# daniel05155/Reinforcement-Learning-in-Music-Generation

Measured on AMD Instinct MI355X. Metric: CW-tokens/sec pretrain fwd+bwd @T=1024, higher is better.
Workload: dtype bf16; 1 GPU; agent_pretrain step (fwd+bwd+clip+Adam), repo dims 512/12/8/2048, synthetic CW tokens (B=512/GPU, T=1024, 7 fields -> 6); per_gpu_batch=512, global_batch=512, seq_len=1024, parallelism=dp1, params=38982227, gemm_table=True

## Files before the change

reinforcement-learning-in-music-generation_amd/csrc/cla_bf16.hip:

```cpp
#include "cwlt_common.h"
#include "cwlt_mfma_bf16.h"

namespace cwlt {
namespace b16 {

__device__ __forceinline__ float phi(float x) { return x > 0.f ? x + 1.f : __expf(x); }
__device__ __forceinline__ float dphi(float x) { return x > 0.f ? 1.f : __expf(x); }
constexpr int FIN_FLOATS = 65 * 64;
__device__ __forceinline__ int stream_of_block(int b, int N, int H) {
    if (N & 7) return b;
    const int x = b & 7, j = b >> 3;
    return ((j / H) * 8 + x) * H + j % H;
}

__device__ __forceinline__ f32x16 load_tile(const float* t, int lane) {
    f32x16 x;
#pragma unroll
    for (int r = 0; r < 16; ++r) x[r] = t[r * 64 + lane];
    return x;
}
__device__ __forceinline__ void store_tile(float* t, int lane, const f32x16& x) {
#pragma unroll
    for (int r = 0; r < 16; ++r) t[r * 64 + lane] = x[r];
}

template <bool STATE_ONLY>
__global__ __launch_bounds__(256) void cla_fwd_bf16_kernel(const bf16_t* __restrict__ q, const bf16_t* __restrict__ k,
                                                           const bf16_t* __restrict__ v, bf16_t* __restrict__ o,
                                                           float* __restrict__ zinv, int H, int L, long ldq, long ldk,
                                                           long ldv, long ldo, float eps, int P, int cps,
                                                           const float* __restrict__ pre, float* __restrict__ part,
                                                           float* __restrict__ fin) {
    __shared__ __attribute__((aligned(16))) bf16_t qs[C * LD];
    __shared__ __attribute__((aligned(16))) bf16_t ks[C * LD];
    __shared__ __attribute__((aligned(16))) bf16_t vs[C * LD];
    __shared__ __attribute__((aligned(16))) bf16_t as_[C * LD];
    __shared__ __attribute__((aligned(16))) float os[C * LDO];
    __shared__ float dens[2][C];

    const int tid = threadIdx.x, lane = tid & 63;
    const int w = __builtin_amdgcn_readfirstlane(tid >> 6);
    const int wi = w >> 1, wj = w & 1;
    const int l31 = lane & 31, hf = lane >> 5;
    const int seg = blockIdx.x % P;
    const int sid = P == 1 ? stream_of_block(blockIdx.x, gridDim.x / H, H) : blockIdx.x / P;
    const int n = sid / H, h = sid % H;
    const bf16_t* qb = q + ((long)n * L) * ldq + h * D;
    const bf16_t* kb = k + ((long)n * L) * ldk + h * D;
    const bf16_t* vb = v + ((long)n * L) * ldv + h * D;
    bf16_t* ob = o + ((long)n * L) * ldo + h * D;
    float* zb = zinv + ((long)n * L) * H + h;

    const int srow = tid >> 3, scol = (tid & 7) * 8;
    const int nch = (L + C - 1) / C;
    const int cbeg = seg * cps, cend = min(nch, cbeg + cps);
    if (cbeg >= nch || (STATE_ONLY && seg == P - 1)) return;
    uint4 rq[2], rk[2], rv[2];
    const bf16x8 ones0 = ones_if(l31 == 0);

    const __amdgpu_buffer_rsrc_t qr = make_rsrc(qb, (uint32_t)(((long)(L - 1) * ldq + D) * 2));
    const __amdgpu_buffer_rsrc_t kr = make_rsrc(kb, (uint32_t)(((long)(L - 1) * ldk + D) * 2));
    const __amdgpu_buffer_rsrc_t vr = make_rsrc(vb, (uint32_t)(((long)(L - 1) * ldv + D) * 2));
#define CLA_LOAD(c)                                                                      \
    _Pragma("unroll") for (int it = 0; it < 2; ++it) {                                   \
        const uint32_t row = (uint32_t)(c) * C + srow + 32 * it;                         \
        if (!STATE_ONLY) rq[it] = buf_load16(qr, (row * (uint32_t)ldq + scol) * 2);      \
        rk[it] = buf_load16(kr, (row * (uint32_t)ldk + scol) * 2);                       \
        rv[it] = buf_load16(vr, (row * (uint32_t)ldv + scol) * 2);                       \
    }
#define CLA_STORE(c)                                                                     \
    _Pragma("unroll") for (int it = 0; it < 2; ++it) {                                   \
        const int row = srow + 32 * it;                                                  \
        const long grow = (long)(c) * C + row;                                           \
        if (grow < L) {                                                                  \
            const float z = 1.0f / (dens[0][row] + dens[1][row] + eps);                  \
            const float4 a = *reinterpret_cast<const float4*>(os + row * LDO + scol);    \
            const float4 b = *reinterpret_cast<const float4*>(os + row * LDO + scol + 4);\
            const float x[8] = {a.x * z, a.y * z, a.z * z, a.w * z, b.x * z, b.y * z, b.z * z, b.w * z}; \
            *reinterpret_cast<uint4*>(ob + grow * ldo + scol) = pack8(x);                \
            if ((tid & 7) == 0) zb[grow * H] = z;                                        \
        }                                                                                \
    }

    CLA_LOAD(cbeg);
    f32x16 S0 = zero16(), S1 = zero16();
    f32x16 Sa = zero16();
    if (!STATE_ONLY && pre && seg > 0) {
        const float* t = pre + (((long)sid * P + seg) * 2 + wj) * (3 * 1024);
        S0 = load_tile(t, lane);
        S1 = load_tile(t + 1024, lane);
        Sa = load_tile(t + 2048, lane);
    }

    for (int c = cbeg; c < cend; ++c) {
        if (!STATE_ONLY && c > cbeg) { CLA_STORE(c - 1); }
#pragma unroll
        for (int it = 0; it < 2; ++it) {
            const int row = srow + 32 * it;
            const bool ok = c * C + row < L;
            float x[8];
            if (!STATE_ONLY) {
                unpack8(rq[it], x);
#pragma unroll
                for (int j = 0; j < 8; ++j) x[j] = ok ? phi(x[j]) : 0.f;
                put_row(qs, row, scol, pack8(x));
            }
            unpack8(rk[it], x);
#pragma unroll
            for (int j = 0; j < 8; ++j) x[j] = ok ? phi(x[j]) : 0.f;
            put_row(ks, row, scol, pack8(x));
            put_row(vs, row, scol, rv[it]);
        }
        __syncthreads();
        if (c + 1 < cend) { CLA_LOAD(c + 1); }

        if (!STATE_ONLY) {
        if (!(wi == 0 && wj == 1)) {
            const f32x16 AT = prod_rows(zero16(), ks, 32 * wj + l31, qs, 32 * wi + l31, 0, 4, hf);
            put_acc_T(as_, 32 * wi + l31, 32 * wj, AT, hf, 0, wi == wj ? l31 : 64, 0.f);
        }
        __syncthreads();

        {
            f32x16 O = zero16(), Oa = zero16();
            const int nks = wi == 0 ? 2 : 4;
#pragma unroll 2
            for (int s = 0; s < nks; ++s) {
                const bf16x8 b = row8(as_, 32 * wi + l31, 16 * s + 8 * hf);
                O = mfma(tfrag8(vs, 16 * s, 32 * wj, lane), b, O);
                if (wj == 0) Oa = mfma(ones0, b, Oa);
            }
#pragma unroll
            for (int t = 0; t < 2; ++t) {
                const f32x16& S = t == 0 ? S0 : S1;
#pragma unroll
                for (int s = 0; s < 2; ++s) {
                    bf16x8 hi, lo;
                    acc_frag(S, s, hi, lo);
                    const bf16x8 b = perm8(qs, 32 * wi + l31, 32 * t + 16 * s, hf);
                    O = mfma_hl(hi, lo, b, O);
                    if (t == wj) {
                        acc_frag(Sa, s, hi, lo);
                        Oa = mfma_hl(hi, lo, b, Oa);
                    }
                }
            }
            put_acc_T_f32(os, 32 * wi + l31, 32 * wj, O, hf);
            if (hf == 0) dens[wj][32 * wi + l31] = Oa[0];
        }
        }
#pragma unroll 2
        for (int s = STATE_ONLY ? 2 * wi : 0; s < (STATE_ONLY ? 2 * wi + 2 : 4); ++s) {
            const bf16x8 b = tfrag8(vs, 16 * s, 32 * wj, lane);
            const bf16x8 a0 = tfrag8(ks, 16 * s, 0, lane);
            const bf16x8 a1 = tfrag8(ks, 16 * s, 32, lane);
            S0 = mfma(a0, b, S0);
            S1 = mfma(a1, b, S1);
            Sa = mfma(wj == 0 ? a0 : a1, ones_if(l31 == 0), Sa);
        }
        __syncthreads();
    }
    if (STATE_ONLY) {
        float* t = part + (((long)sid * P + seg) * 4 + w) * (3 * 1024);
        store_tile(t, lane, S0);
        store_tile(t + 1024, lane, S1);
        store_tile(t + 2048, lane, Sa);
        return;
    }
    CLA_STORE(cend - 1);
#undef CLA_LOAD
#undef CLA_STORE
    if (fin) {
        __syncthreads();
        if (wi == 0) {
            put_acc_T_f32(os, 32 * wj + l31, 0, S0, hf);
            put_acc_T_f32(os, 32 * wj + l31, 32, S1, hf);
            if (l31 == 0) {
#pragma unroll
                for (int r = 0; r < 16; ++r) dens[0][32 * wj + acc_row(r, hf)] = Sa[r];
            }
        }
        __syncthreads();
        float* f = fin + (long)sid * FIN_FLOATS;
#pragma unroll
        for (int it = 0; it < 4; ++it) {
            const int row = (tid >> 4) + 16 * it, col = (tid & 15) * 4;
            *reinterpret_cast<float4*>(f + row * 64 + col) = *reinterpret_cast<const float4*>(os + row * LDO + col);
        }
        if (tid < 64) f[64 * 64 + tid] = dens[0][tid];
    }
}

__global__ __launch_bounds__(256) void seg_prefix_kernel(const float* __restrict__ part, float* __restrict__ pre,
                                                         long total, int P, int NT, int nfwd) {
    const long i = (long)blockIdx.x * 256 + threadIdx.x;
    if (i >= total) return;
    const int e = (int)(i & 1023);
    const int tile = (int)((i >> 10) % NT);
    const int wj = (int)((i >> 10) / NT) & 1;
    const long sid = (i >> 10) / NT / 2;
    const long pstride = (long)4 * NT * 1024, ostride = (long)2 * NT * 1024;
    const float* a = part + sid * P * pstride + ((long)wj * NT + tile) * 1024 + e;
    const float* b = a + (long)2 * NT * 1024;
    float* o = pre + sid * P * ostride + ((long)wj * NT + tile) * 1024 + e;
    float run = 0.f;
    if (tile < nfwd) {
        for (int p = 0; p < P; ++p) {
            o[p * ostride] = run;
            if (p < P - 1) run += a[p * pstride] + b[p * pstride];
        }
    } else {
        for (int p = P - 1; p >= 0; --p) {
            o[p * ostride] = run;
            if (p > 0) run += a[p * pstride] + b[p * pstride];
        }
    }
}

__device__ __forceinline__ uint4 stage_g(uint4 rdo, uint4 ro, float z, float& dden) {
    float a[8], b[8];
    unpack8(rdo, a);
    unpack8(ro, b);
    float dot = 0.f;
#pragma unroll
    for (int j = 0; j < 8; ++j) {
        dot = fmaf(a[j], b[j], dot);
        a[j] *= z;
    }
    dot += dpp_move<0xB1>(dot);
    dot += dpp_move<0x4E>(dot);
    dot += dpp_move<0x141>(dot);
    dden = -dot * z;
    return pack8(a);
}

__device__ __forceinline__ void colsum_store(float (&bsum)[8], float* scratch, float* dst, int tid, int lane, int w) {
    __syncthreads();
#pragma unroll
    for (int j = 0; j < 8; ++j) {
        float v = bsum[j];
        v += __shfl_xor(v, 8, 64);
        v += __shfl_xor(v, 16, 64);
        v += __shfl_xor(v, 32, 64);
        if ((lane >> 3) == 0) scratch[w * 64 + (lane & 7) * 8 + j] = v;
    }
    __syncthreads();
    if (tid < 64) dst[tid] = (scratch[tid] + scratch[64 + tid]) + (scratch[128 + tid] + scratch[192 + tid]);
}

template <bool HAS_DDEN>
__global__ __launch_bounds__(256) void cla_bwd_dq_bf16_kernel(
    const bf16_t* __restrict__ q, const bf16_t* __restrict__ k, const bf16_t* __restrict__ v,
    const bf16_t* __restrict__ out, const bf16_t* __restrict__ dout, const float* __restrict__ zinv,
    const float* __restrict__ dden_in, bf16_t* __restrict__ dq, float* __restrict__ csum, int H, int L, long ldq,
    long ldk, long ldv, long ldo, long lddo, long lddq, int P, int cps, const float* __restrict__ pre) {
    __shared__ __attribute__((aligned(16))) bf16_t gs[C * LD];
    __shared__ __attribute__((aligned(16))) bf16_t vs[C * LD];
    __shared__ __attribute__((aligned(16))) bf16_t ks[C * LD];
    __shared__ __attribute__((aligned(16))) bf16_t ws[C * LD];
    __shared__ __attribute__((aligned(16))) float os[C * LDO];
    __shared__ float dd[C];

    const int tid = threadIdx.x, lane = tid & 63;
    const int w = __builtin_amdgcn_readfirstlane(tid >> 6);
    const int wi = w >> 1, wj = w & 1;
    const int l31 = lane & 31, hf = lane >> 5;
    const int sid = blockIdx.x / P, seg = blockIdx.x % P;
    const int n = sid / H, h = sid % H;
    const bf16_t* qb = q + ((long)n * L) * ldq + h * D;
    const bf16_t* kb = k + ((long)n * L) * ldk + h * D;
    const bf16_t* vb = v + ((long)n * L) * ldv + h * D;
    const bf16_t* ob = out + ((long)n * L) * ldo + h * D;
    const bf16_t* gb = dout + ((long)n * L) * lddo + h * D;
    const float* zb = zinv + ((long)n * L) * H + h;
    const float* ddb = HAS_DDEN ? dden_in + ((long)n * L) * H + h : zb;
    bf16_t* dqb = dq + ((long)n * L) * lddq + h * D;

    const int srow = tid >> 3, scol = (tid & 7) * 8;
    const int nch = (L + C - 1) / C;
    const int cbeg = seg * cps, cend = min(nch, cbeg + cps);
    if (cbeg >= nch) return;
    uint4 rq[2], rk[2], rv[2], rg[2], ro[2], rqp[2];
    float rz[2], rdd[2];

    const __amdgpu_buffer_rsrc_t qr = make_rsrc(qb, (uint32_t)(((long)(L - 1) * ldq + D) * 2));
    const __amdgpu_buffer_rsrc_t kr = make_rsrc(kb, (uint32_t)(((long)(L - 1) * ldk + D) * 2));
    const __amdgpu_buffer_rsrc_t vr = make_rsrc(vb, (uint32_t)(((long)(L - 1) * ldv + D) * 2));
    const __amdgpu_buffer_rsrc_t gr = make_rsrc(gb, (uint32_t)(((long)(L - 1) * lddo + D) * 2));
    const __amdgpu_buffer_rsrc_t orr = make_rsrc(ob, (uint32_t)(((long)(L - 1) * ldo + D) * 2));
    const __amdgpu_buffer_rsrc_t zr = make_rsrc(zb, (uint32_t)(((long)(L - 1) * H + 1) * 4));
    const __amdgpu_buffer_rsrc_t ddr = make_rsrc(ddb, (uint32_t)(((long)(L - 1) * H + 1) * 4));
#define CLA_LOAD(c)                                                                      \
    _Pragma("unroll") for (int it = 0; it < 2; ++it) {                                   \
        const uint32_t row = (uint32_t)(c) * C + srow + 32 * it;                         \
        rq[it] = buf_load16(qr, (row * (uint32_t)ldq + scol) * 2);                       \
        rk[it] = buf_load16(kr, (row * (uint32_t)ldk + scol) * 2);                       \
        rv[it] = buf_load16(vr, (row * (uint32_t)ldv + scol) * 2);                       \
        rg[it] = buf_load16(gr, (row * (uint32_t)lddo + scol) * 2);                      \
        rz[it] = __builtin_bit_cast(float, __builtin_amdgcn_raw_buffer_load_b32(zr, (int)(row * (uint32_t)H * 4), 0, 0)); \
        if (HAS_DDEN)                                                                    \
            rdd[it] = __builtin_bit_cast(float, __builtin_amdgcn_raw_buffer_load_b32(ddr, (int)(row * (uint32_t)H * 4), 0, 0)); \
        else                                                                             \
            ro[it] = buf_load16(orr, (row * (uint32_t)ldo + scol) * 2);                  \
    }
#define CLA_STORE(c)                                                                     \
    _Pragma("unroll") for (int it = 0; it < 2; ++it) {                                   \
        const int row = srow + 32 * it;                                                  \
        const long grow = (long)(c) * C + row;                                           \
        if (grow < L) {                                                                  \
            const float4 a = *reinterpret_cast<const float4*>(os + row * LDO + scol);    \
            const float4 b = *reinterpret_cast<const float4*>(os + row * LDO + scol + 4);\
            float x[8];                                                                  \
            unpack8(rqp[it], x);                                                         \
            x[0] = a.x * dphi(x[0]); x[1] = a.y * dphi(x[1]); x[2] = a.z * dphi(x[2]);   \
            x[3] = a.w * dphi(x[3]); x[4] = b.x * dphi(x[4]); x[5] = b.y * dphi(x[5]);   \
            x[6] = b.z * dphi(x[6]); x[7] = b.w * dphi(x[7]);                            \
            _Pragma("unroll") for (int j = 0; j < 8; ++j) bsum[j] += x[j];               \
            *reinterpret_cast<uint4*>(dqb + grow * lddq + scol) = pack8(x);              \
        }                                                                                \
    }

    float bsum[8];
#pragma unroll
    for (int j = 0; j < 8; ++j) bsum[j] = 0.f;
    CLA_LOAD(cbeg);
    f32x16 T0 = zero16(), T1 = zero16();
    f32x16 Ta = zero16();
    if (pre && seg > 0) {
        const float* t = pre + (((long)sid * P + seg) * 2 + wj) * (8 * 1024);
        T0 = load_tile(t, lane);
        T1 = load_tile(t + 1024, lane);
        Ta = load_tile(t + 2048, lane);
    }
    const bf16x8 ones0 = ones_if(l31 == 0);

    for (int c = cbeg; c < cend; ++c) {
        if (c > cbeg) { CLA_STORE(c - 1); }
#pragma unroll
        for (int it = 0; it < 2; ++it) {
            const int row = srow + 32 * it;
            const bool ok = c * C + row < L;
            float dden;
            uint4 gp;
            if (HAS_DDEN) {
                float a[8];
                unpack8(rg[it], a);
#pragma unroll
                for (int j = 0; j < 8; ++j) a[j] *= rz[it];
                gp = pack8(a);
                dden = rdd[it];
            } else {
                gp = stage_g(rg[it], ro[it], rz[it], dden);
            }
            if ((tid & 7) == 0) dd[row] = dden;
            put_row(gs, row, scol, gp);
            put_row(vs, row, scol, rv[it]);
            float x[8];
            unpack8(rk[it], x);
#pragma unroll
            for (int j = 0; j < 8; ++j) x[j] = ok ? phi(x[j]) : 0.f;
            put_row(ks, row, scol, pack8(x));
            rqp[it] = rq[it];
        }
        __syncthreads();
        if (c + 1 < cend) { CLA_LOAD(c + 1); }

        const float dden_i = dd[32 * wi + l31];
        if (!(wi == 0 && wj == 1)) {
            const f32x16 WT = prod_rows(zero16(), vs, 32 * wj + l31, gs, 32 * wi + l31, 0, 4, hf);
            put_acc_T(ws, 32 * wi + l31, 32 * wj, WT, hf, 0, wi == wj ? l31 : 64, dden_i);
        }
        __syncthreads();

        {
            f32x16 Q = zero16();
            const int nks = wi == 0 ? 2 : 4;
#pragma unroll 2
            for (int s = 0; s < nks; ++s)
                Q = mfma(tfrag8(ks, 16 * s, 32 * wj, lane), row8(ws, 32 * wi + l31, 16 * s + 8 * hf), Q);
            Q = prod_accA(Q, T0, T1, gs, 32 * wi + l31, hf);
            {
                bf16x8 hi, lo;
                acc_frag(Ta, 0, hi, lo);
                const bf16x8 b = first_if(hf == 0, dden_i);
                Q = mfma_hl(hi, lo, b, Q);
            }
            put_acc_T_f32(os, 32 * wi + l31, 32 * wj, Q, hf);
        }
#pragma unroll 2
        for (int s = 0; s < 4; ++s) {
            const bf16x8 b = tfrag8(ks, 16 * s, 32 * wj, lane);
            T0 = mfma(tfrag8(vs, 16 * s, 0, lane), b, T0);
            T1 = mfma(tfrag8(vs, 16 * s, 32, lane), b, T1);
            Ta = mfma(ones0, b, Ta);
        }
        __syncthreads();
    }
    CLA_STORE(cend - 1);
#undef CLA_LOAD
#undef CLA_STORE
    if (csum) colsum_store(bsum, os, csum + (((long)n * P + seg) * H + h) * D, tid, lane, w);
}

template <bool STATE_ONLY>
__global__ __launch_bounds__(256, 2) void cla_bwd_dkdv_bf16_kernel(
    const bf16_t* __restrict__ q, const bf16_t* __restrict__ k, const bf16_t* __restrict__ v,
    const bf16_t* __restrict__ out, const bf16_t* __restrict__ dout, const float* __restrict__ zinv,
    bf16_t* __restrict__ dk, bf16_t* __restrict__ dv, float* __restrict__ csum_k, float* __restrict__ csum_v,
    float* __restrict__ dden_out, int H, int L, long ldq, long ldk, long ldv, long ldo, long lddo, long lddk,
    long lddv, int P, int cps, const float* __restrict__ pre, float* __restrict__ part) {
    __shared__ __attribute__((aligned(16))) bf16_t qs[C * LD];
    __shared__ __attribute__((aligned(16))) bf16_t ks[C * LD];
    __shared__ __attribute__((aligned(16))) bf16_t vs[C * LD];
    __shared__ __attribute__((aligned(16))) bf16_t gs[C * LD];
    __shared__ __attribute__((aligned(16))) bf16_t wt[C * LD];
    __shared__ __attribute__((aligned(16))) bf16_t at[C * LD];
    __shared__ __attribute__((aligned(16))) bf16_t ok_[C * LD];
    __shared__ __attribute__((aligned(16))) bf16_t ov[C * LD];
    __shared__ float dd[C];

    const int tid = threadIdx.x, lane = tid & 63;
    const int w = __builtin_amdgcn_readfirstlane(tid >> 6);
    const int wi = w >> 1, wj = w & 1;
    const int l31 = lane & 31, hf = lane >> 5;
    const int sid = blockIdx.x / P, seg = blockIdx.x % P;
    const int n = sid / H, h = sid % H;
    const bf16_t* qb = q + ((long)n * L) * ldq + h * D;
    const bf16_t* kb = k + ((long)n * L) * ldk + h * D;
    const bf16_t* vb = v + ((long)n * L) * ldv + h * D;
    const bf16_t* ob = out + ((long)n * L) * ldo + h * D;
    const bf16_t* gb = dout + ((long)n * L) * lddo + h * D;
    const float* zb = zinv + ((long)n * L) * H + h;
    bf16_t* dkb = dk + ((long)n * L) * lddk + h * D;
    bf16_t* dvb = dv + ((long)n * L) * lddv + h * D;
    float* ddb = dden_out ? dden_out + ((long)n * L) * H + h : nullptr;

    const int srow = tid >> 3, scol = (tid & 7) * 8;
    const int nch = (L + C - 1) / C;
    const int cbeg = seg * cps, cend = min(nch, cbeg + cps);
    if (cbeg >= nch) return;
    uint4 rq[2], rk[2], rv[2], rg[2], ro[2];
    float rz[2];

    const __amdgpu_buffer_rsrc_t qr = make_rsrc(qb, (uint32_t)(((long)(L - 1) * ldq + D) * 2));
    const __amdgpu_buffer_rsrc_t kr = make_rsrc(kb, (uint32_t)(((long)(L - 1) * ldk + D) * 2));
    const __amdgpu_buffer_rsrc_t vr = make_rsrc(vb, (uint32_t)(((long)(L - 1) * ldv + D) * 2));
    const __amdgpu_buffer_rsrc_t gr = make_rsrc(gb, (uint32_t)(((long)(L - 1) * lddo + D) * 2));
    const __amdgpu_buffer_rsrc_t orr = make_rsrc(ob, (uint32_t)(((long)(L - 1) * ldo + D) * 2));
    const __amdgpu_buffer_rsrc_t zr = make_rsrc(zb, (uint32_t)(((long)(L - 1) * H + 1) * 4));
#define CLA_LOAD(c)                                                                      \
    _Pragma("unroll") for (int it = 0; it < 2; ++it) {                                   \
        const uint32_t row = (uint32_t)(c) * C + srow + 32 * it;                         \
        rq[it] = buf_load16(qr, (row * (uint32_t)ldq + scol) * 2);                       \
        rk[it] = buf_load16(kr, (row * (uint32_t)ldk + scol) * 2);                       \
        rv[it] = buf_load16(vr, (row * (uint32_t)ldv + scol) * 2);                       \
        rg[it] = buf_load16(gr, (row * (uint32_t)lddo + scol) * 2);                      \
        ro[it] = buf_load16(orr, (row * (uint32_t)ldo + scol) * 2);                      \
        rz[it] = __builtin_bit_cast(float, __builtin_amdgcn_raw_buffer_load_b32(zr, (int)(row * (uint32_t)H * 4), 0, 0)); \
    }
#define CLA_STORE(c)                                                                     \
    _Pragma("unroll") for (int it = 0; it < 2; ++it) {                                   \
        const int row = srow + 32 * it;                                                  \
        const long grow = (long)(c) * C + row;                                           \
        if (grow < L) {                                                                  \
            float x[8], f[8];                                                            \
            unpack8(*reinterpret_cast<const uint4*>(ok_ + row * LD + scol), x);          \
            unpack8(*reinterpret_cast<const uint4*>(ks + row * LD + scol), f);           \
            _Pragma("unroll") for (int j = 0; j < 8; ++j) x[j] *= fminf(f[j], 1.0f);     \
            _Pragma("unroll") for (int j = 0; j < 8; ++j) bsk[j] += x[j];                \
            *reinterpret_cast<uint4*>(dkb + grow * lddk + scol) = pack8(x);              \
            const uint4 vv = *reinterpret_cast<const uint4*>(ov + row * LD + scol);      \
            unpack8(vv, f);                                                              \
            _Pragma("unroll") for (int j = 0; j < 8; ++j) bsv[j] += f[j];                \
            *reinterpret_cast<uint4*>(dvb + grow * lddv + scol) = vv;                    \
        }                                                                                \
    }

    float bsk[8], bsv[8];
#pragma unroll
    for (int j = 0; j < 8; ++j) bsk[j] = bsv[j] = 0.f;

    CLA_LOAD(cend - 1);
    f32x16 RT0 = zero16(), RT1 = zero16();
    f32x16 RTa = zero16();
    f32x16 R20 = zero16(), R21 = zero16();
    f32x16 T0 = zero16(), T1 = zero16(), Ta = zero16();
    const bf16x8 ones0 = ones_if(l31 == 0);
    if (!STATE_ONLY && pre && seg < P - 1) {
        const float* t = pre + (((long)sid * P + seg) * 2 + wj) * (8 * 1024) + 3 * 1024;
        RT0 = load_tile(t, lane);
        RT1 = load_tile(t + 1024, lane);
        RTa = load_tile(t + 2048, lane);
        R20 = load_tile(t + 3072, lane);
        R21 = load_tile(t + 4096, lane);
    }

    for (int c = cend - 1; c >= cbeg; --c) {
        if (!STATE_ONLY && c < cend - 1) { CLA_STORE(c + 1); }
#pragma unroll
        for (int it = 0; it < 2; ++it) {
            const int row = srow + 32 * it;
            const bool ok = c * C + row < L;
            float dden;
            const uint4 gp = stage_g(rg[it], ro[it], rz[it], dden);
            if ((tid & 7) == 0) {
                dd[row] = dden;
                if (!STATE_ONLY && ddb && ok) ddb[((long)c * C + row) * H] = dden;
            }
            put_row(gs, row, scol, gp);
            put_row(vs, row, scol, rv[it]);
            float x[8];
            unpack8(rk[it], x);
#pragma unroll
            for (int j = 0; j < 8; ++j) x[j] = ok ? phi(x[j]) : 0.f;
            put_row(ks, row, scol, pack8(x));
            unpack8(rq[it], x);
#pragma unroll
            for (int j = 0; j < 8; ++j) x[j] = ok ? phi(x[j]) : 0.f;
            put_row(qs, row, scol, pack8(x));
        }
        __syncthreads();
        if (c > cbeg) { CLA_LOAD(c - 1); }

        if (!STATE_ONLY) {
        if (!(wi == 0 && wj == 1)) {
            f32x16 W = prod_rows(zero16(), gs, 32 * wi + l31, vs, 32 * wj + l31, 0, 4, hf);
            W = mfma(first_if(hf == 0, dd[32 * wi + l31]), first_if(hf == 0, 1.0f), W);
            put_acc_T(wt, 32 * wj + l31, 32 * wi, W, hf, wi == wj ? l31 : 0, 64, 0.f);
            const f32x16 A = prod_rows(zero16(), qs, 32 * wi + l31, ks, 32 * wj + l31, 0, 4, hf);
            put_acc_T(at, 32 * wj + l31, 32 * wi, A, hf, wi == wj ? l31 : 0, 64, 0.f);
        }
        __syncthreads();

        {
            const int s0 = wi == 1 ? 2 : 0;
            f32x16 K = zero16();
#pragma unroll 2
            for (int s = s0; s < 4; ++s)
                K = mfma(tfrag8(qs, 16 * s, 32 * wj, lane), row8(wt, 32 * wi + l31, 16 * s + 8 * hf), K);
            K = prod_accA(K, RT0, RT1, vs, 32 * wi + l31, hf);
            {
                bf16x8 hi, lo;
                acc_frag(RTa, 0, hi, lo);
                const bf16x8 b = first_if(hf == 0, 1.0f);
                K = mfma_hl(hi, lo, b, K);
            }
            put_acc_T(ok_, 32 * wi + l31, 32 * wj, K, hf, 0, 64, 0.f);
            f32x16 V = zero16();
#pragma unroll 2
            for (int s = s0; s < 4; ++s)
                V = mfma(tfrag8(gs, 16 * s, 32 * wj, lane), row8(at, 32 * wi + l31, 16 * s + 8 * hf), V);
            V = prod_accA(V, R20, R21, ks, 32 * wi + l31, hf);
            put_acc_T(ov, 32 * wi + l31, 32 * wj, V, hf, 0, 64, 0.f);
        }
        }
#pragma unroll 2
        for (int s = STATE_ONLY ? 2 * wi : 0; s < (STATE_ONLY ? 2 * wi + 2 : 4); ++s) {
            const bf16x8 g0 = tfrag8(gs, 16 * s, 0, lane), g1 = tfrag8(gs, 16 * s, 32, lane);
            const bf16x8 q0 = tfrag8(qs, 16 * s, 0, lane), q1 = tfrag8(qs, 16 * s, 32, lane);
            const bf16x8 bq = wj == 0 ? q0 : q1;
            const bf16x8 bg = wj == 0 ? g0 : g1;
            RT0 = mfma(g0, bq, RT0);
            RT1 = mfma(g1, bq, RT1);
            R20 = mfma(q0, bg, R20);
            R21 = mfma(q1, bg, R21);
            bf16x8 dh, dl;
#pragma unroll
            for (int j = 0; j < 8; ++j) {
                const float x = l31 == 0 ? dd[16 * s + 8 * hf + j] : 0.f;
                const __bf16 hh = (__bf16)x;
                dh[j] = hh;
                dl[j] = (__bf16)(x - (float)hh);
            }
            RTa = mfma(dh, bq, RTa);
            RTa = mfma(dl, bq, RTa);
            if (STATE_ONLY) {
                const bf16x8 bk = tfrag8(ks, 16 * s, 32 * wj, lane);
                T0 = mfma(tfrag8(vs, 16 * s, 0, lane), bk, T0);
                T1 = mfma(tfrag8(vs, 16 * s, 32, lane), bk, T1);
                Ta = mfma(ones0, bk, Ta);
            }
        }
        __syncthreads();
    }
    if (STATE_ONLY) {
        float* t = part + (((long)sid * P + seg) * 4 + w) * (8 * 1024);
        store_tile(t, lane, T0);
        store_tile(t + 1024, lane, T1);
        store_tile(t + 2048, lane, Ta);
        store_tile(t + 3072, lane, RT0);
        store_tile(t + 4096, lane, RT1);
        store_tile(t + 5120, lane, RTa);
        store_tile(t + 6144, lane, R20);
        store_tile(t + 7168, lane, R21);
        return;
    }
    CLA_STORE(cbeg);
#undef CLA_LOAD
#undef CLA_STORE
    if (csum_k) {
        float* scratch = reinterpret_cast<float*>(wt);
        colsum_store(bsk, scratch, csum_k + (((long)n * P + seg) * H + h) * D, tid, lane, w);
        colsum_store(bsv, scratch, csum_v + (((long)n * P + seg) * H + h) * D, tid, lane, w);
    }
}

struct ChunkRegs {
    uint4 q, k, v, g, o;
    float z;
};

__device__ __forceinline__ float min1(float f) { return __builtin_amdgcn_fmed3f(f, 0.0f, 1.0f); }

__device__ __forceinline__ void put_acc_T_dphi(bf16_t* x, const bf16_t* f_t, int xrow, int c0, const f32x16& acc, int hf) {
#pragma unroll
    for (int g = 0; g < 4; ++g) {
        const uint2 fr = *reinterpret_cast<const uint2*>(f_t + xrow * LD + c0 + 8 * g + 4 * hf);
        const float f0 = __uint_as_float(fr.x << 16), f1 = __uint_as_float(fr.x & 0xffff0000u);
        const float f2 = __uint_as_float(fr.y << 16), f3 = __uint_as_float(fr.y & 0xffff0000u);
        bf16x4 p;
        p[0] = (__bf16)(acc[4 * g] * min1(f0));
        p[1] = (__bf16)(acc[4 * g + 1] * min1(f1));
        p[2] = (__bf16)(acc[4 * g + 2] * min1(f2));
        p[3] = (__bf16)(acc[4 * g + 3] * min1(f3));
        *reinterpret_cast<uint2*>(x + xrow * LD + c0 + 8 * g + 4 * hf) = __builtin_bit_cast(uint2, p);
    }
}
__device__ __forceinline__ void put_acc_T_all(bf16_t* x, int xrow, int c0, const f32x16& acc, int hf) {
#pragma unroll
    for (int g = 0; g < 4; ++g) {
        bf16x4 p;
#pragma unroll
        for (int u = 0; u < 4; ++u) p[u] = (__bf16)acc[4 * g + u];
        *reinterpret_cast<uint2*>(x + xrow * LD + c0 + 8 * g + 4 * hf) = __builtin_bit_cast(uint2, p);
    }
}
__device__ __forceinline__ void put_acc_T_ge(bf16_t* x, int xrow, int c0, const f32x16& acc, int hf, int lo) {
#pragma unroll
    for (int g = 0; g < 4; ++g) {
        bf16x4 p;
#pragma unroll
        for (int u = 0; u < 4; ++u) p[u] = (__bf16)(8 * g + 4 * hf + u >= lo ? acc[4 * g + u] : 0.f);
        *reinterpret_cast<uint2*>(x + xrow * LD + c0 + 8 * g + 4 * hf) = __builtin_bit_cast(uint2, p);
    }
}
__device__ __forceinline__ f32x16 prod_rows4(const bf16_t* a_t, int arow, const bf16_t* b_t, int brow, int hf) {
    f32x16 acc = mfma(row8(a_t, arow, 8 * hf), row8(b_t, brow, 8 * hf), zero16());
#pragma unroll
    for (int s = 1; s < 4; ++s) acc = mfma(row8(a_t, arow, 16 * s + 8 * hf), row8(b_t, brow, 16 * s + 8 * hf), acc);
    return acc;
}
__device__ __forceinline__ bf16x8 negate8(bf16x8 x) {
    uint4 u = __builtin_bit_cast(uint4, x);
    u.x ^= 0x80008000u; u.y ^= 0x80008000u; u.z ^= 0x80008000u; u.w ^= 0x80008000u;
    return __builtin_bit_cast(bf16x8, u);
}

__global__ __launch_bounds__(512, 1) void cla_bwd_sweep_bf16_kernel(
    const bf16_t* __restrict__ q, const bf16_t* __restrict__ k, const bf16_t* __restrict__ v,
    const bf16_t* __restrict__ out, const bf16_t* __restrict__ dout, const float* __restrict__ zinv,
    const float* __restrict__ fin, bf16_t* __restrict__ dq, bf16_t* __restrict__ dk, bf16_t* __restrict__ dv,
    float* __restrict__ csum_q, float* __restrict__ csum_k, float* __restrict__ csum_v, int H, int L, long ldq,
    long ldk, long ldv, long ldo, long lddo, long lddq, long lddk, long lddv) {
    constexpr int TILE = C * LD;
    __shared__ __attribute__((aligned(16))) bf16_t in_[2 * 4 * TILE];
    __shared__ __attribute__((aligned(16))) bf16_t er[2 * TILE];
    __shared__ __attribute__((aligned(16))) bf16_t es[TILE];
    __shared__ __attribute__((aligned(16))) bf16_t wt[TILE];
    __shared__ __attribute__((aligned(16))) bf16_t at[TILE];
    __shared__ __attribute__((aligned(16))) bf16_t ok_[TILE];
    __shared__ __attribute__((aligned(16))) bf16_t ov[TILE];
    __shared__ __attribute__((aligned(16))) bf16_t oq[TILE];
    __shared__ float dd[2][C];
    __shared__ float r1s[2][C];
    __shared__ float ksm[C];

    const int tid = threadIdx.x, lane = tid & 63;
    const int w8 = __builtin_amdgcn_readfirstlane(tid >> 6);
    const bool kvg = w8 < 4;
    const int w = w8 & 3, wi = w >> 1, wj = w & 1;
    const int l31 = lane & 31, hf = lane >> 5;
    const int sid = stream_of_block(blockIdx.x, gridDim.x / H, H);
    const int n = sid / H, h = sid % H;
    const bf16_t* qb = q + ((long)n * L) * ldq + h * D;
    const bf16_t* kb = k + ((long)n * L) * ldk + h * D;
    const bf16_t* vb = v + ((long)n * L) * ldv + h * D;
    const bf16_t* ob = out + ((long)n * L) * ldo + h * D;
    const bf16_t* gb = dout + ((long)n * L) * lddo + h * D;
    const float* zb = zinv + ((long)n * L) * H + h;
    bf16_t* dqb = dq + ((long)n * L) * lddq + h * D;
    bf16_t* dkb = dk + ((long)n * L) * lddk + h * D;
    bf16_t* dvb = dv + ((long)n * L) * lddv + h * D;

    const int srow = tid >> 3, scol = (tid & 7) * 8;
    const int orow = (tid & 255) >> 3;
    const int nch = (L + C - 1) / C;

    const __amdgpu_buffer_rsrc_t qr = make_rsrc(qb, (uint32_t)(((long)(L - 1) * ldq + D) * 2));
    const __amdgpu_buffer_rsrc_t kr = make_rsrc(kb, (uint32_t)(((long)(L - 1) * ldk + D) * 2));
    const __amdgpu_buffer_rsrc_t vr = make_rsrc(vb, (uint32_t)(((long)(L - 1) * ldv + D) * 2));
    const __amdgpu_buffer_rsrc_t gr = make_rsrc(gb, (uint32_t)(((long)(L - 1) * lddo + D) * 2));
    const __amdgpu_buffer_rsrc_t orr = make_rsrc(ob, (uint32_t)(((long)(L - 1) * ldo + D) * 2));
    const __amdgpu_buffer_rsrc_t zr = make_rsrc(zb, (uint32_t)(((long)(L - 1) * H + 1) * 4));

    auto load = [&](ChunkRegs& R, int c) __attribute__((always_inline)) {
        const uint32_t row = (uint32_t)c * C + srow;
        R.q = buf_load16(qr, (row * (uint32_t)ldq + scol) * 2);
        R.k = buf_load16(kr, (row * (uint32_t)ldk + scol) * 2);
        R.v = buf_load16(vr, (row * (uint32_t)ldv + scol) * 2);
        R.g = buf_load16(gr, (row * (uint32_t)lddo + scol) * 2);
        R.o = buf_load16(orr, (row * (uint32_t)ldo + scol) * 2);
        R.z = __builtin_bit_cast(float, __builtin_amdgcn_raw_buffer_load_b32(zr, (int)(row * (uint32_t)H * 4), 0, 0));
    };
    auto stage = [&](const ChunkRegs& R, int c, int b) __attribute__((always_inline)) {
        bf16_t* t = in_ + b * 4 * TILE;
        float dden;
        const uint4 gp = stage_g(R.g, R.o, R.z, dden);
        put_row(t + 3 * TILE, srow, scol, gp);
        if ((tid & 7) == 0) {
            dd[b][srow] = dden;
            const __bf16 hh = (__bf16)dden;
            const __bf16 ll = (__bf16)(dden - (float)hh);
            const uint32_t hl = (uint32_t)__builtin_bit_cast(unsigned short, hh) |
                                ((uint32_t)__builtin_bit_cast(unsigned short, ll) << 16);
            put_row(t + 3 * TILE, srow, 64, make_uint4(hl, 0u, 0u, 0u));
        }
        put_row(t + 2 * TILE, srow, scol, R.v);
        float x[8], y[8];
        unpack8(R.k, x);
        unpack8(R.q, y);
#pragma unroll
        for (int j = 0; j < 8; ++j) {
            x[j] = phi(x[j]);
            y[j] = phi(y[j]);
        }
        if ((c + 1) * C > L && c * C + srow >= L) {
#pragma unroll
            for (int j = 0; j < 8; ++j) x[j] = y[j] = 0.f;
        }
        put_row(t + 1 * TILE, srow, scol, pack8(x));
        put_row(t, srow, scol, pack8(y));
    };

    typedef float f32x8 __attribute__((ext_vector_type(8)));
    f32x8 bs0 = 0.f, bs1 = 0.f;
    auto widen = [](uint4 r) __attribute__((always_inline)) {
        f32x8 x;
        x[0] = __uint_as_float(r.x << 16); x[1] = __uint_as_float(r.x & 0xffff0000u);
        x[2] = __uint_as_float(r.y << 16); x[3] = __uint_as_float(r.y & 0xffff0000u);
        x[4] = __uint_as_float(r.z << 16); x[5] = __uint_as_float(r.z & 0xffff0000u);
        x[6] = __uint_as_float(r.w << 16); x[7] = __uint_as_float(r.w & 0xffff0000u);
        return x;
    };
    const bf16_t* t0 = kvg ? ok_ : oq;
    bf16_t* g0 = kvg ? dkb : dqb;
    const long l0 = kvg ? lddk : lddq;
    auto store = [&](int c, f32x8& b0, f32x8& b1) __attribute__((always_inline)) {
#pragma unroll
        for (int it = 0; it < 2; ++it) {
            const int row = orow + 32 * it;
            const long grow = (long)c * C + row;
            if (grow < L) {
                const uint4 a = *reinterpret_cast<const uint4*>(t0 + row * LD + scol);
                b0 += widen(a);
                *reinterpret_cast<uint4*>(g0 + grow * l0 + scol) = a;
                if (kvg) {
                    const uint4 b = *reinterpret_cast<const uint4*>(ov + row * LD + scol);
                    b1 += widen(b);
                    *reinterpret_cast<uint4*>(dvb + grow * lddv + scol) = b;
                }
            }
        }
    };

    f32x16 st = zero16(), sa = zero16();
    if (!kvg) {
        const float* f = fin + (long)sid * FIN_FLOATS;
#pragma unroll
        for (int r = 0; r < 16; ++r) st[r] = f[(32 * wi + acc_row(r, hf)) * 64 + 32 * wj + l31];
        if (wi == 0) sa[0] = hf == 0 ? f[64 * 64 + 32 * wj + l31] : 0.f;
    } else {
        put_acc_T_all(er, 32 * wj + l31, 32 * wi, st, hf);
        if (wi == 0 && hf == 0) r1s[0][32 * wj + l31] = 0.f;
    }
    const bf16x8 ones0 = ones_if(l31 == 0);
    const bf16x8 one0 = first_if(hf == 0, 1.0f);

    auto iter = [&](int c, ChunkRegs& R, const int b) __attribute__((always_inline)) {
        if (c < nch - 1) store(c + 1, bs0, bs1);
        if (c >= 1) {
            stage(R, c - 1, 1 - b);
            if (c >= 3) load(R, c - 3);
        }
        const bf16_t* qs = in_ + b * 4 * TILE;
        const bf16_t* ks = qs + TILE;
        const bf16_t* vs = qs + 2 * TILE;
        const bf16_t* gs = qs + 3 * TILE;
        const float dden_i = dd[b][32 * wi + l31];
        __builtin_amdgcn_sched_barrier(0);
        if (kvg) {
            if (!(wi == 0 && wj == 1)) {
                f32x16 W = prod_rows4(gs, 32 * wi + l31, vs, 32 * wj + l31, hf);
                W = mfma(first_if(hf == 0, dden_i), one0, W);
                if (wi == wj) put_acc_T_ge(wt, 32 * wj + l31, 32 * wi, W, hf, l31);
                else put_acc_T_all(wt, 32 * wj + l31, 32 * wi, W, hf);
            }
            __builtin_amdgcn_sched_barrier(0);
#pragma unroll
            for (int s = 0; s < 4; ++s) {
                const bf16x8 bq = tfrag8(qs, 16 * s, 32 * wj, lane);
                st = mfma(tfrag8(gs, 16 * s, 32 * wi, lane), bq, st);
                if (wi == 0) sa = mfma(tfrag8(gs, 16 * s, 64, lane), bq, sa);
            }
            if (c > 0) {
                put_acc_T_all(er + (1 - b) * TILE, 32 * wj + l31, 32 * wi, st, hf);
                if (wi == 0 && hf == 0) r1s[1 - b][32 * wj + l31] = sa[0] + sa[1];
            }
        } else {
            if (!(wi == 0 && wj == 1)) {
                const f32x16 A = prod_rows4(qs, 32 * wi + l31, ks, 32 * wj + l31, hf);
                if (wi == wj) put_acc_T_ge(at, 32 * wj + l31, 32 * wi, A, hf, l31);
                else put_acc_T_all(at, 32 * wj + l31, 32 * wi, A, hf);
            }
            __builtin_amdgcn_sched_barrier(0);
            if (c == 0) {
                st = zero16();
                sa = zero16();
            } else {
#pragma unroll
                for (int s = 0; s < 4; ++s) {
                    const bf16x8 nb = negate8(tfrag8(ks, 16 * s, 32 * wj, lane));
                    st = mfma(tfrag8(vs, 16 * s, 32 * wi, lane), nb, st);
                    if (wi == 0) sa = mfma(ones0, nb, sa);
                }
            }
            put_acc_T_all(es, 32 * wj + l31, 32 * wi, st, hf);
            if (wi == 0 && hf == 0) ksm[32 * wj + l31] = sa[0];
        }
        __syncthreads();
        if (kvg) {
            const bf16_t* rs = er + b * TILE;
            f32x16 K = prod_rows4(rs, 32 * wj + l31, vs, 32 * wi + l31, hf);
            K = mfma(first_if(hf == 0, r1s[b][32 * wj + l31]), one0, K);
            f32x16 V = mfma(tfrag8(rs, 0, 32 * wj, lane), row8(ks, 32 * wi + l31, 8 * hf), zero16());
#pragma unroll
            for (int s = 1; s < 4; ++s)
                V = mfma(tfrag8(rs, 16 * s, 32 * wj, lane), row8(ks, 32 * wi + l31, 16 * s + 8 * hf), V);
            __builtin_amdgcn_sched_barrier(0);
            if (wi == 0) {
#pragma unroll
                for (int s = 0; s < 2; ++s) {
                    K = mfma(tfrag8(qs, 16 * s, 32 * wj, lane), row8(wt, 32 * wi + l31, 16 * s + 8 * hf), K);
                    V = mfma(tfrag8(gs, 16 * s, 32 * wj, lane), row8(at, 32 * wi + l31, 16 * s + 8 * hf), V);
                }
            }
#pragma unroll
            for (int s = 2; s < 4; ++s) {
                K = mfma(tfrag8(qs, 16 * s, 32 * wj, lane), row8(wt, 32 * wi + l31, 16 * s + 8 * hf), K);
                V = mfma(tfrag8(gs, 16 * s, 32 * wj, lane), row8(at, 32 * wi + l31, 16 * s + 8 * hf), V);
            }
            __builtin_amdgcn_sched_barrier(0);
            put_acc_T_dphi(ok_, ks, 32 * wi + l31, 32 * wj, K, hf);
            put_acc_T_all(ov, 32 * wi + l31, 32 * wj, V, hf);
        } else {
            f32x16 Q = prod_rows4(es, 32 * wj + l31, gs, 32 * wi + l31, hf);
            Q = mfma(first_if(hf == 0, ksm[32 * wj + l31]), first_if(hf == 0, dden_i), Q);
            __builtin_amdgcn_sched_barrier(0);
#pragma unroll
            for (int s = 0; s < 2; ++s)
                Q = mfma(tfrag8(ks, 16 * s, 32 * wj, lane), tfrag8(wt, 16 * s, 32 * wi, lane), Q);
            if (wi == 1) {
#pragma unroll
                for (int s = 2; s < 4; ++s)
                    Q = mfma(tfrag8(ks, 16 * s, 32 * wj, lane), tfrag8(wt, 16 * s, 32 * wi, lane), Q);
            }
            put_acc_T_dphi(oq, qs, 32 * wi + l31, 32 * wj, Q, hf);
        }
        __syncthreads();
    };

    ChunkRegs RA, RB;
    load(RA, nch - 1);
    if (nch > 1) load(RB, nch - 2);
    stage(RA, nch - 1, 0);
    if (nch > 2) load(RA, nch - 3);
    __syncthreads();
    for (int c = nch - 1; c >= 0; c -= 2) {
        iter(c, RB, 0);
        if (c >= 1) iter(c - 1, RA, 1);
    }
    store(0, bs0, bs1);

    if (csum_q) {
        float* scratch = reinterpret_cast<float*>(wt);
        __syncthreads();
#pragma unroll
        for (int j = 0; j < 8; ++j) {
            float x = bs0[j], y = bs1[j];
            x += __shfl_xor(x, 8, 64);
            y += __shfl_xor(y, 8, 64);
            x += __shfl_xor(x, 16, 64);
            y += __shfl_xor(y, 16, 64);
            x += __shfl_xor(x, 32, 64);
            y += __shfl_xor(y, 32, 64);
            if ((lane >> 3) == 0) {
                scratch[((kvg ? 1 : 0) * 4 + w) * 64 + (lane & 7) * 8 + j] = x;
                if (kvg) scratch[(2 * 4 + w) * 64 + (lane & 7) * 8 + j] = y;
            }
        }
        __syncthreads();
        if (tid < 192) {
            const int a = tid >> 6, e = tid & 63;
            const float s = (scratch[(a * 4 + 0) * 64 + e] + scratch[(a * 4 + 1) * 64 + e]) +
                            (scratch[(a * 4 + 2) * 64 + e] + scratch[(a * 4 + 3) * 64 + e]);
            float* dst = a == 0 ? csum_q : a == 1 ? csum_k : csum_v;
            dst[(long)sid * D + e] = s;
        }
    }
}

}

int scan_segments(int N, int H, int L) {
    const long streams = (long)N * H;
    const int nch = (L + b16::C - 1) / b16::C;
    if (streams >= 256 || nch < 4) return 1;
    long want = (512 + streams - 1) / streams;
    if (want > 16) want = 16;
    if (want > nch / 2) want = nch / 2;
    if (want < 2) return 1;
    const int cps = (nch + (int)want - 1) / (int)want;
    return (nch + cps - 1) / cps;
}
static int seg_cps(int L, int P) { return (((L + b16::C - 1) / b16::C) + P - 1) / P; }

long scan_seg_floats(int N, int H, int P, int backward) {
    return P > 1 ? (long)N * H * P * 6 * (backward ? 8 : 3) * 1024 : 0;
}

long scan_final_state_floats(int N, int H) { return (long)N * H * b16::FIN_FLOATS; }

int launch_cla_fwd_bf16(const void* q, const void* k, const void* v, void* out, float* zinv, int N, int H, int L,
                        long ldq, long ldk, long ldv, long ldo, float eps, int P, float* ws, float* fin,
                        hipStream_t st) {
    const int nch = (L + b16::C - 1) / b16::C;
    if (P <= 1) {
        hipLaunchKernelGGL(b16::cla_fwd_bf16_kernel<false>, dim3(N * H), dim3(256), 0, st, (const bf16_t*)q,
                           (const bf16_t*)k, (const bf16_t*)v, (bf16_t*)out, zinv, H, L, ldq, ldk, ldv, ldo, eps, 1, nch,
                           (const float*)nullptr, (float*)nullptr, fin);
        return (int)hipGetLastError();
    }
    const int cps = seg_cps(L, P);
    const long NS = (long)N * H;
    float* part = ws;
    float* pre = ws + NS * P * 4 * 3 * 1024;
    hipLaunchKernelGGL(b16::cla_fwd_bf16_kernel<true>, dim3(NS * P), dim3(256), 0, st, (const bf16_t*)q,
                       (const bf16_t*)k, (const bf16_t*)v, (bf16_t*)out, zinv, H, L, ldq, ldk, ldv, ldo, eps, P, cps,
                       (const float*)nullptr, part, (float*)nullptr);
    const long total = NS * 2 * 3 * 1024;
    hipLaunchKernelGGL(b16::seg_prefix_kernel, dim3((unsigned)((total + 255) / 256)), dim3(256), 0, st, part, pre, total,
                       P, 3, 3);
    hipLaunchKernelGGL(b16::cla_fwd_bf16_kernel<false>, dim3(NS * P), dim3(256), 0, st, (const bf16_t*)q,
                       (const bf16_t*)k, (const bf16_t*)v, (bf16_t*)out, zinv, H, L, ldq, ldk, ldv, ldo, eps, P, cps,
                       (const float*)pre, (float*)nullptr, (float*)nullptr);
    return (int)hipGetLastError();
}

int launch_cla_bwd_sweep_bf16(const void* q, const void* k, const void* v, const void* out, const float* zinv,
                              const void* dout, const float* fin, void* dq, void* dk, void* dv, float* csum_q,
                              float* csum_k, float* csum_v, int N, int H, int L, long ldq, long ldk, long ldv, long ldo,
                              long lddo, long lddq, long lddk, long lddv, hipStream_t st) {
    hipLaunchKernelGGL(b16::cla_bwd_sweep_bf16_kernel, dim3(N * H), dim3(512), 0, st, (const bf16_t*)q,
                       (const bf16_t*)k, (const bf16_t*)v, (const bf16_t*)out, (const bf16_t*)dout, zinv, fin,
                       (bf16_t*)dq, (bf16_t*)dk, (bf16_t*)dv, csum_q, csum_k, csum_v, H, L, ldq, ldk, ldv, ldo, lddo,
                       lddq, lddk, lddv);
    return (int)hipGetLastError();
}

int launch_cla_bwd_dq_bf16(const void* q, const void* k, const void* v, const void* out, const float* zinv,
                           const void* dout, const float* dden, void* dq, float* csum, int N, int H, int L, long ldq,
                           long ldk, long ldv, long ldo, long lddo, long lddq, int P, float* ws, hipStream_t st) {
    const int nch = (L + b16::C - 1) / b16::C;
    const long NS = (long)N * H;
    const int cps = P > 1 ? seg_cps(L, P) : nch;
    const float* pre = P > 1 ? ws + NS * P * 4 * 8 * 1024 : nullptr;
    if (P < 1) P = 1;
    if (dden)
        hipLaunchKernelGGL(b16::cla_bwd_dq_bf16_kernel<true>, dim3(NS * P), dim3(256), 0, st, (const bf16_t*)q,
                           (const bf16_t*)k, (const bf16_t*)v, (const bf16_t*)out, (const bf16_t*)dout, zinv, dden,
                           (bf16_t*)dq, csum, H, L, ldq, ldk, ldv, ldo, lddo, lddq, P, cps, pre);
    else
        hipLaunchKernelGGL(b16::cla_bwd_dq_bf16_kernel<false>, dim3(NS * P), dim3(256), 0, st, (const bf16_t*)q,
                           (const bf16_t*)k, (const bf16_t*)v, (const bf16_t*)out, (const bf16_t*)dout, zinv, dden,
                           (bf16_t*)dq, csum, H, L, ldq, ldk, ldv, ldo, lddo, lddq, P, cps, pre);
    return (int)hipGetLastError();
}

int launch_cla_bwd_dkdv_bf16(const void* q, const void* k, const void* v, const void* out, const float* zinv,
                             const void* dout, void* dk, void* dv, float* csum_k, float* csum_v, float* dden_out,
                             int N, int H, int L, long ldq, long ldk, long ldv, long ldo, long lddo, long lddk,
                             long lddv, int P, float* ws, hipStream_t st) {
    const int nch = (L + b16::C - 1) / b16::C;
    const long NS = (long)N * H;
    if (P <= 1) {
        hipLaunchKernelGGL(b16::cla_bwd_dkdv_bf16_kernel<false>, dim3(NS), dim3(256), 0, st, (const bf16_t*)q,
                           (const bf16_t*)k, (const bf16_t*)v, (const bf16_t*)out, (const bf16_t*)dout, zinv,
                           (bf16_t*)dk, (bf16_t*)dv, csum_k, csum_v, dden_out, H, L, ldq, ldk, ldv, ldo, lddo, lddk,
                           lddv, 1, nch, (const float*)nullptr, (float*)nullptr);
        return (int)hipGetLastError();
    }
    const int cps = seg_cps(L, P);
    float* part = ws;
    float* pre = ws + NS * P * 4 * 8 * 1024;
    hipLaunchKernelGGL(b16::cla_bwd_dkdv_bf16_kernel<true>, dim3(NS * P), dim3(256), 0, st, (const bf16_t*)q,
                       (const bf16_t*)k, (const bf16_t*)v, (const bf16_t*)out, (const bf16_t*)dout, zinv, (bf16_t*)dk,
                       (bf16_t*)dv, (float*)nullptr, (float*)nullptr, (float*)nullptr, H, L, ldq, ldk, ldv, ldo, lddo,
                       lddk, lddv, P, cps, (const float*)nullptr, part);
    const long total = NS * 2 * 8 * 1024;
    hipLaunchKernelGGL(b16::seg_prefix_kernel, dim3((unsigned)((total + 255) / 256)), dim3(256), 0, st, part, pre, total,
                       P, 8, 3);
    hipLaunchKernelGGL(b16::cla_bwd_dkdv_bf16_kernel<false>, dim3(NS * P), dim3(256), 0, st, (const bf16_t*)q,
                       (const bf16_t*)k, (const bf16_t*)v, (const bf16_t*)out, (const bf16_t*)dout, zinv, (bf16_t*)dk,
                       (bf16_t*)dv, csum_k, csum_v, dden_out, H, L, ldq, ldk, ldv, ldo, lddo, lddk, lddv, P, cps,
                       (const float*)pre, (float*)nullptr);
    return (int)hipGetLastError();
}

}
```

reinforcement-learning-in-music-generation_amd/csrc/cwlt_mfma_bf16.h:

```cpp
#pragma once
#include "cwlt_common.h"

namespace cwlt {
namespace b16 {

constexpr int D = 64;
constexpr int C = 64;
constexpr int LD = 72;
constexpr int LDO = 68;

typedef __bf16 bf16x8 __attribute__((ext_vector_type(8)));
typedef __bf16 bf16x4 __attribute__((ext_vector_type(4)));
typedef short s16x4 __attribute__((ext_vector_type(4)));
typedef __attribute__((address_space(3))) s16x4 lds_s16x4;

__device__ __forceinline__ constexpr int acc_row(int r, int hf) { return (r & 3) + 8 * (r >> 2) + 4 * hf; }

__device__ __forceinline__ f32x16 mfma(bf16x8 a, bf16x8 b, f32x16 c) {
    return __builtin_amdgcn_mfma_f32_32x32x16_bf16(a, b, c, 0, 0, 0);
}
__device__ __forceinline__ f32x16 zero16() {
    f32x16 z;
#pragma unroll
    for (int i = 0; i < 16; ++i) z[i] = 0.f;
    return z;
}

__device__ __forceinline__ bf16x8 row8(const bf16_t* t, int row, int k) {
    return __builtin_bit_cast(bf16x8, *reinterpret_cast<const uint4*>(t + row * LD + k));
}
__device__ __forceinline__ bf16x8 perm8(const bf16_t* t, int row, int k0, int hf) {
    const uint2 a = *reinterpret_cast<const uint2*>(t + row * LD + k0 + 4 * hf);
    const uint2 b = *reinterpret_cast<const uint2*>(t + row * LD + k0 + 8 + 4 * hf);
    return __builtin_bit_cast(bf16x8, make_uint4(a.x, a.y, b.x, b.y));
}
__device__ __forceinline__ bf16x8 tfrag8(const bf16_t* t, int k0, int c0, int lane) {
    const int q = (lane >> 2) & 3, p = lane & 3;
    const bf16_t* base = t + (k0 + 8 * (lane >> 5) + q) * LD + c0 + 16 * ((lane >> 4) & 1) + 4 * p;
    const s16x4 a = __builtin_amdgcn_ds_read_tr16_b64_v4i16((lds_s16x4*)(base));
    const s16x4 b = __builtin_amdgcn_ds_read_tr16_b64_v4i16((lds_s16x4*)(base + 4 * LD));
    return __builtin_bit_cast(bf16x8, __builtin_shufflevector(a, b, 0, 1, 2, 3, 4, 5, 6, 7));
}
#ifndef CWLT_STATE_LO
#define CWLT_STATE_LO 0
#endif
constexpr bool STATE_LO = CWLT_STATE_LO != 0;
__device__ __forceinline__ f32x16 mfma_hl(const bf16x8& hi, const bf16x8& lo, bf16x8 b, f32x16 acc) {
    acc = __builtin_amdgcn_mfma_f32_32x32x16_bf16(hi, b, acc, 0, 0, 0);
    if (STATE_LO) acc = __builtin_amdgcn_mfma_f32_32x32x16_bf16(lo, b, acc, 0, 0, 0);
    return acc;
}
__device__ __forceinline__ void acc_frag(const f32x16& S, int s, bf16x8& hi, bf16x8& lo) {
#pragma unroll
    for (int j = 0; j < 8; ++j) {
        const float x = S[8 * s + j];
        const __bf16 h = (__bf16)x;
        hi[j] = h;
        lo[j] = (__bf16)(x - (float)h);
    }
}
__device__ __forceinline__ bf16x8 first_if(bool c, float x) {
    bf16x8 v;
#pragma unroll
    for (int j = 0; j < 8; ++j) v[j] = (__bf16)0.0f;
    v[0] = (__bf16)(c ? x : 0.0f);
    return v;
}
__device__ __forceinline__ bf16x8 ones_if(bool c) {
    bf16x8 v;
#pragma unroll
    for (int j = 0; j < 8; ++j) v[j] = (__bf16)(c ? 1.0f : 0.0f);
    return v;
}

__device__ __forceinline__ f32x16 prod_rows(f32x16 acc, const bf16_t* a_t, int arow, const bf16_t* b_t, int brow,
                                            int s0, int s1, int hf) {
#pragma unroll 2
    for (int s = s0; s < s1; ++s)
        acc = mfma(row8(a_t, arow, 16 * s + 8 * hf), row8(b_t, brow, 16 * s + 8 * hf), acc);
    return acc;
}
__device__ __forceinline__ f32x16 prod_accA(f32x16 acc, const f32x16& X0, const f32x16& X1, const bf16_t* b_t,
                                            int brow, int hf) {
#pragma unroll
    for (int t = 0; t < 2; ++t) {
        const f32x16& X = t == 0 ? X0 : X1;
#pragma unroll
        for (int s = 0; s < 2; ++s) {
            bf16x8 hi, lo;
            acc_frag(X, s, hi, lo);
            const bf16x8 b = perm8(b_t, brow, 32 * t + 16 * s, hf);
            acc = mfma_hl(hi, lo, b, acc);
        }
    }
    return acc;
}

__device__ __forceinline__ void unpack8(uint4 r, float (&x)[8]) {
    x[0] = __uint_as_float(r.x << 16); x[1] = __uint_as_float(r.x & 0xffff0000u);
    x[2] = __uint_as_float(r.y << 16); x[3] = __uint_as_float(r.y & 0xffff0000u);
    x[4] = __uint_as_float(r.z << 16); x[5] = __uint_as_float(r.z & 0xffff0000u);
    x[6] = __uint_as_float(r.w << 16); x[7] = __uint_as_float(r.w & 0xffff0000u);
}
__device__ __forceinline__ uint4 pack8(const float (&x)[8]) {
    bf16x8 v;
#pragma unroll
    for (int j = 0; j < 8; ++j) v[j] = (__bf16)x[j];
    return __builtin_bit_cast(uint4, v);
}
__device__ __forceinline__ void put_row(bf16_t* t, int row, int col, uint4 v) {
    *reinterpret_cast<uint4*>(t + row * LD + col) = v;
}
__device__ __forceinline__ void put_acc_T(bf16_t* x, int xrow, int c0, const f32x16& acc, int hf, int lo, int hi,
                                          float add) {
#pragma unroll
    for (int g = 0; g < 4; ++g) {
        bf16x4 p;
#pragma unroll
        for (int u = 0; u < 4; ++u) {
            const int rr = 8 * g + 4 * hf + u;
            p[u] = (__bf16)((rr >= lo && rr <= hi) ? acc[4 * g + u] + add : 0.f);
        }
        *reinterpret_cast<uint2*>(x + xrow * LD + c0 + 8 * g + 4 * hf) = __builtin_bit_cast(uint2, p);
    }
}
__device__ __forceinline__ void put_acc_T_f32(float* x, int xrow, int c0, const f32x16& acc, int hf) {
#pragma unroll
    for (int g = 0; g < 4; ++g)
        *reinterpret_cast<float4*>(x + xrow * LDO + c0 + 8 * g + 4 * hf) =
            make_float4(acc[4 * g], acc[4 * g + 1], acc[4 * g + 2], acc[4 * g + 3]);
}

}
}
```

Baseline: 3.254 million CW-tokens/s.

## Swizzle LDS tiles with XOR layout and software-pipeline MFMA fragment fetches

```diff
diff --git a/reinforcement-learning-in-music-generation_amd/csrc/cla_bf16.hip b/reinforcement-learning-in-music-generation_amd/csrc/cla_bf16.hip
--- a/reinforcement-learning-in-music-generation_amd/csrc/cla_bf16.hip
+++ b/reinforcement-learning-in-music-generation_amd/csrc/cla_bf16.hip
@@ -1,3 +1,5 @@
+#include <type_traits>
+
 #include "cwlt_common.h"
 #include "cwlt_mfma_bf16.h"
 
@@ -31,10 +33,10 @@
                                                            long ldv, long ldo, float eps, int P, int cps,
                                                            const float* __restrict__ pre, float* __restrict__ part,
                                                            float* __restrict__ fin) {
-    __shared__ __attribute__((aligned(16))) bf16_t qs[C * LD];
-    __shared__ __attribute__((aligned(16))) bf16_t ks[C * LD];
-    __shared__ __attribute__((aligned(16))) bf16_t vs[C * LD];
-    __shared__ __attribute__((aligned(16))) bf16_t as_[C * LD];
+    __shared__ __attribute__((aligned(16))) bf16_t qs[sw::TILE];
+    __shared__ __attribute__((aligned(16))) bf16_t ks[sw::TILE];
+    __shared__ __attribute__((aligned(16))) bf16_t vs[sw::TILE];
+    __shared__ __attribute__((aligned(16))) bf16_t as_[sw::TILE];
     __shared__ __attribute__((aligned(16))) float os[C * LDO];
     __shared__ float dens[2][C];
 
@@ -52,6 +54,13 @@
     float* zb = zinv + ((long)n * L) * H + h;
 
     const int srow = tid >> 3, scol = (tid & 7) * 8;
+    int sb = sw::base(srow, scol);
+    int bi8 = sw::base(32 * wi + l31, 8 * hf), bj8 = sw::base(32 * wj + l31, 8 * hf);
+    int bi4 = sw::base(32 * wi + l31, 4 * hf), bj4 = sw::base(32 * wj + l31, 4 * hf);
+    sw::TBase tb = sw::tbase(lane);
+#define CLA_FRESH()                                                                                  \
+    CWLT_SW_FRESH(sb); CWLT_SW_FRESH(bi8); CWLT_SW_FRESH(bj8); CWLT_SW_FRESH(bi4); CWLT_SW_FRESH(bj4); \
+    CWLT_SW_FRESH(tb.b0); CWLT_SW_FRESH(tb.b4)
     const int nch = (L + C - 1) / C;
     const int cbeg = seg * cps, cend = min(nch, cbeg + cps);
     if (cbeg >= nch || (STATE_ONLY && seg == P - 1)) return;
@@ -93,6 +102,7 @@
     }
 
     for (int c = cbeg; c < cend; ++c) {
+        CLA_FRESH();
         if (!STATE_ONLY && c > cbeg) { CLA_STORE(c - 1); }
 #pragma unroll
         for (int it = 0; it < 2; ++it) {
@@ -103,21 +113,21 @@
                 unpack8(rq[it], x);
 #pragma unroll
                 for (int j = 0; j < 8; ++j) x[j] = ok ? phi(x[j]) : 0.f;
-                put_row(qs, row, scol, pack8(x));
+                sw::put_row(qs + 32 * it * sw::ROW, sb, pack8(x));
             }
             unpack8(rk[it], x);
 #pragma unroll
             for (int j = 0; j < 8; ++j) x[j] = ok ? phi(x[j]) : 0.f;
-            put_row(ks, row, scol, pack8(x));
-            put_row(vs, row, scol, rv[it]);
+            sw::put_row(ks + 32 * it * sw::ROW, sb, pack8(x));
+            sw::put_row(vs + 32 * it * sw::ROW, sb, rv[it]);
         }
         __syncthreads();
         if (c + 1 < cend) { CLA_LOAD(c + 1); }
 
         if (!STATE_ONLY) {
         if (!(wi == 0 && wj == 1)) {
-            const f32x16 AT = prod_rows(zero16(), ks, 32 * wj + l31, qs, 32 * wi + l31, 0, 4, hf);
-            put_acc_T(as_, 32 * wi + l31, 32 * wj, AT, hf, 0, wi == wj ? l31 : 64, 0.f);
+            const f32x16 AT = sw::prod_rows(zero16(), ks, bj8, qs, bi8, 0, 4);
+            sw::put_acc_T(as_, bi4, 32 * wj, AT, hf, 0, wi == wj ? l31 : 64, 0.f);
         }
         __syncthreads();
 
@@ -126,8 +136,8 @@
             const int nks = wi == 0 ? 2 : 4;
 #pragma unroll 2
             for (int s = 0; s < nks; ++s) {
-                const bf16x8 b = row8(as_, 32 * wi + l31, 16 * s + 8 * hf);
-                O = mfma(tfrag8(vs, 16 * s, 32 * wj, lane), b, O);
+                const bf16x8 b = sw::row8(as_, bi8, 16 * s);
+                O = mfma(sw::tfrag8(vs, tb, 16 * s, 32 * wj), b, O);
                 if (wj == 0) Oa = mfma(ones0, b, Oa);
             }
 #pragma unroll
@@ -137,7 +147,7 @@
                 for (int s = 0; s < 2; ++s) {
                     bf16x8 hi, lo;
                     acc_frag(S, s, hi, lo);
-                    const bf16x8 b = perm8(qs, 32 * wi + l31, 32 * t + 16 * s, hf);
+                    const bf16x8 b = sw::perm8(qs, bi4, 32 * t + 16 * s);
                     O = mfma_hl(hi, lo, b, O);
                     if (t == wj) {
                         acc_frag(Sa, s, hi, lo);
@@ -151,9 +161,9 @@
         }
 #pragma unroll 2
         for (int s = STATE_ONLY ? 2 * wi : 0; s < (STATE_ONLY ? 2 * wi + 2 : 4); ++s) {
-            const bf16x8 b = tfrag8(vs, 16 * s, 32 * wj, lane);
-            const bf16x8 a0 = tfrag8(ks, 16 * s, 0, lane);
-            const bf16x8 a1 = tfrag8(ks, 16 * s, 32, lane);
+            const bf16x8 b = sw::tfrag8(vs, tb, 16 * s, 32 * wj);
+            const bf16x8 a0 = sw::tfrag8(ks, tb, 16 * s, 0);
+            const bf16x8 a1 = sw::tfrag8(ks, tb, 16 * s, 32);
             S0 = mfma(a0, b, S0);
             S1 = mfma(a1, b, S1);
             Sa = mfma(wj == 0 ? a0 : a1, ones_if(l31 == 0), Sa);
@@ -170,6 +180,7 @@
     CLA_STORE(cend - 1);
 #undef CLA_LOAD
 #undef CLA_STORE
+#undef CLA_FRESH
     if (fin) {
         __syncthreads();
         if (wi == 0) {
@@ -254,10 +265,10 @@
     const bf16_t* __restrict__ out, const bf16_t* __restrict__ dout, const float* __restrict__ zinv,
     const float* __restrict__ dden_in, bf16_t* __restrict__ dq, float* __restrict__ csum, int H, int L, long ldq,
     long ldk, long ldv, long ldo, long lddo, long lddq, int P, int cps, const float* __restrict__ pre) {
-    __shared__ __attribute__((aligned(16))) bf16_t gs[C * LD];
-    __shared__ __attribute__((aligned(16))) bf16_t vs[C * LD];
-    __shared__ __attribute__((aligned(16))) bf16_t ks[C * LD];
-    __shared__ __attribute__((aligned(16))) bf16_t ws[C * LD];
+    __shared__ __attribute__((aligned(16))) bf16_t gs[sw::TILE];
+    __shared__ __attribute__((aligned(16))) bf16_t vs[sw::TILE];
+    __shared__ __attribute__((aligned(16))) bf16_t ks[sw::TILE];
+    __shared__ __attribute__((aligned(16))) bf16_t ws[sw::TILE];
     __shared__ __attribute__((aligned(16))) float os[C * LDO];
     __shared__ float dd[C];
 
@@ -277,6 +288,13 @@
     bf16_t* dqb = dq + ((long)n * L) * lddq + h * D;
 
     const int srow = tid >> 3, scol = (tid & 7) * 8;
+    int sb = sw::base(srow, scol);
+    int bi8 = sw::base(32 * wi + l31, 8 * hf), bj8 = sw::base(32 * wj + l31, 8 * hf);
+    int bi4 = sw::base(32 * wi + l31, 4 * hf), bj4 = sw::base(32 * wj + l31, 4 * hf);
+    sw::TBase tb = sw::tbase(lane);
+#define CLA_FRESH()                                                                                  \
+    CWLT_SW_FRESH(sb); CWLT_SW_FRESH(bi8); CWLT_SW_FRESH(bj8); CWLT_SW_FRESH(bi4); CWLT_SW_FRESH(bj4); \
+    CWLT_SW_FRESH(tb.b0); CWLT_SW_FRESH(tb.b4)
     const int nch = (L + C - 1) / C;
     const int cbeg = seg * cps, cend = min(nch, cbeg + cps);
     if (cbeg >= nch) return;
@@ -335,6 +353,7 @@
     const bf16x8 ones0 = ones_if(l31 == 0);
 
     for (int c = cbeg; c < cend; ++c) {
+        CLA_FRESH();
         if (c > cbeg) { CLA_STORE(c - 1); }
 #pragma unroll
         for (int it = 0; it < 2; ++it) {
@@ -353,13 +372,13 @@
                 gp = stage_g(rg[it], ro[it], rz[it], dden);
             }
             if ((tid & 7) == 0) dd[row] = dden;
-            put_row(gs, row, scol, gp);
-            put_row(vs, row, scol, rv[it]);
+            sw::put_row(gs + 32 * it * sw::ROW, sb, gp);
+            sw::put_row(vs + 32 * it * sw::ROW, sb, rv[it]);
             float x[8];
             unpack8(rk[it], x);
 #pragma unroll
             for (int j = 0; j < 8; ++j) x[j] = ok ? phi(x[j]) : 0.f;
-            put_row(ks, row, scol, pack8(x));
+            sw::put_row(ks + 32 * it * sw::ROW, sb, pack8(x));
             rqp[it] = rq[it];
         }
         __syncthreads();
@@ -367,8 +386,8 @@
 
         const float dden_i = dd[32 * wi + l31];
         if (!(wi == 0 && wj == 1)) {
-            const f32x16 WT = prod_rows(zero16(), vs, 32 * wj + l31, gs, 32 * wi + l31, 0, 4, hf);
-            put_acc_T(ws, 32 * wi + l31, 32 * wj, WT, hf, 0, wi == wj ? l31 : 64, dden_i);
+            const f32x16 WT = sw::prod_rows(zero16(), vs, bj8, gs, bi8, 0, 4);
+            sw::put_acc_T(ws, bi4, 32 * wj, WT, hf, 0, wi == wj ? l31 : 64, dden_i);
         }
         __syncthreads();
 
@@ -377,8 +396,8 @@
             const int nks = wi == 0 ? 2 : 4;
 #pragma unroll 2
             for (int s = 0; s < nks; ++s)
-                Q = mfma(tfrag8(ks, 16 * s, 32 * wj, lane), row8(ws, 32 * wi + l31, 16 * s + 8 * hf), Q);
-            Q = prod_accA(Q, T0, T1, gs, 32 * wi + l31, hf);
+                Q = mfma(sw::tfrag8(ks, tb, 16 * s, 32 * wj), sw::row8(ws, bi8, 16 * s), Q);
+            Q = sw::prod_accA(Q, T0, T1, gs, bi4);
             {
                 bf16x8 hi, lo;
                 acc_frag(Ta, 0, hi, lo);
@@ -389,9 +408,9 @@
         }
 #pragma unroll 2
         for (int s = 0; s < 4; ++s) {
-            const bf16x8 b = tfrag8(ks, 16 * s, 32 * wj, lane);
-            T0 = mfma(tfrag8(vs, 16 * s, 0, lane), b, T0);
-            T1 = mfma(tfrag8(vs, 16 * s, 32, lane), b, T1);
+            const bf16x8 b = sw::tfrag8(ks, tb, 16 * s, 32 * wj);
+            T0 = mfma(sw::tfrag8(vs, tb, 16 * s, 0), b, T0);
+            T1 = mfma(sw::tfrag8(vs, tb, 16 * s, 32), b, T1);
             Ta = mfma(ones0, b, Ta);
         }
         __syncthreads();
@@ -399,6 +418,7 @@
     CLA_STORE(cend - 1);
 #undef CLA_LOAD
 #undef CLA_STORE
+#undef CLA_FRESH
     if (csum) colsum_store(bsum, os, csum + (((long)n * P + seg) * H + h) * D, tid, lane, w);
 }
 
@@ -409,14 +429,14 @@
     bf16_t* __restrict__ dk, bf16_t* __restrict__ dv, float* __restrict__ csum_k, float* __restrict__ csum_v,
     float* __restrict__ dden_out, int H, int L, long ldq, long ldk, long ldv, long ldo, long lddo, long lddk,
     long lddv, int P, int cps, const float* __restrict__ pre, float* __restrict__ part) {
-    __shared__ __attribute__((aligned(16))) bf16_t qs[C * LD];
-    __shared__ __attribute__((aligned(16))) bf16_t ks[C * LD];
-    __shared__ __attribute__((aligned(16))) bf16_t vs[C * LD];
-    __shared__ __attribute__((aligned(16))) bf16_t gs[C * LD];
-    __shared__ __attribute__((aligned(16))) bf16_t wt[C * LD];
-    __shared__ __attribute__((aligned(16))) bf16_t at[C * LD];
-    __shared__ __attribute__((aligned(16))) bf16_t ok_[C * LD];
-    __shared__ __attribute__((aligned(16))) bf16_t ov[C * LD];
+    __shared__ __attribute__((aligned(16))) bf16_t qs[sw::TILE];
+    __shared__ __attribute__((aligned(16))) bf16_t ks[sw::TILE];
+    __shared__ __attribute__((aligned(16))) bf16_t vs[sw::TILE];
+    __shared__ __attribute__((aligned(16))) bf16_t gs[sw::TILE];
+    __shared__ __attribute__((aligned(16))) bf16_t wt[sw::TILE];
+    __shared__ __attribute__((aligned(16))) bf16_t at[sw::TILE];
+    __shared__ __attribute__((aligned(16))) bf16_t ok_[sw::TILE];
+    __shared__ __attribute__((aligned(16))) bf16_t ov[sw::TILE];
     __shared__ float dd[C];
 
     const int tid = threadIdx.x, lane = tid & 63;
@@ -436,6 +456,13 @@
     float* ddb = dden_out ? dden_out + ((long)n * L) * H + h : nullptr;
 
     const int srow = tid >> 3, scol = (tid & 7) * 8;
+    int sb = sw::base(srow, scol);
+    int bi8 = sw::base(32 * wi + l31, 8 * hf), bj8 = sw::base(32 * wj + l31, 8 * hf);
+    int bi4 = sw::base(32 * wi + l31, 4 * hf), bj4 = sw::base(32 * wj + l31, 4 * hf);
+    sw::TBase tb = sw::tbase(lane);
+#define CLA_FRESH()                                                                                  \
+    CWLT_SW_FRESH(sb); CWLT_SW_FRESH(bi8); CWLT_SW_FRESH(bj8); CWLT_SW_FRESH(bi4); CWLT_SW_FRESH(bj4); \
+    CWLT_SW_FRESH(tb.b0); CWLT_SW_FRESH(tb.b4)
     const int nch = (L + C - 1) / C;
     const int cbeg = seg * cps, cend = min(nch, cbeg + cps);
     if (cbeg >= nch) return;
@@ -464,12 +491,12 @@
         const long grow = (long)(c) * C + row;                                           \
         if (grow < L) {                                                                  \
             float x[8], f[8];                                                            \
-            unpack8(*reinterpret_cast<const uint4*>(ok_ + row * LD + scol), x);          \
-            unpack8(*reinterpret_cast<const uint4*>(ks + row * LD + scol), f);           \
+            unpack8(sw::get_row(ok_ + 32 * it * sw::ROW, sb), x);                        \
+            unpack8(sw::get_row(ks + 32 * it * sw::ROW, sb), f);                         \
             _Pragma("unroll") for (int j = 0; j < 8; ++j) x[j] *= fminf(f[j], 1.0f);     \
             _Pragma("unroll") for (int j = 0; j < 8; ++j) bsk[j] += x[j];                \
             *reinterpret_cast<uint4*>(dkb + grow * lddk + scol) = pack8(x);              \
-            const uint4 vv = *reinterpret_cast<const uint4*>(ov + row * LD + scol);      \
+            const uint4 vv = sw::get_row(ov + 32 * it * sw::ROW, sb);                    \
             unpack8(vv, f);                                                              \
             _Pragma("unroll") for (int j = 0; j < 8; ++j) bsv[j] += f[j];                \
             *reinterpret_cast<uint4*>(dvb + grow * lddv + scol) = vv;                    \
@@ -496,6 +523,7 @@
     }
 
     for (int c = cend - 1; c >= cbeg; --c) {
+        CLA_FRESH();
         if (!STATE_ONLY && c < cend - 1) { CLA_STORE(c + 1); }
 #pragma unroll
         for (int it = 0; it < 2; ++it) {
@@ -507,28 +535,28 @@
                 dd[row] = dden;
                 if (!STATE_ONLY && ddb && ok) ddb[((long)c * C + row) * H] = dden;
             }
-            put_row(gs, row, scol, gp);
-            put_row(vs, row, scol, rv[it]);
+            sw::put_row(gs + 32 * it * sw::ROW, sb, gp);
+            sw::put_row(vs + 32 * it * sw::ROW, sb, rv[it]);
             float x[8];
             unpack8(rk[it], x);
 #pragma unroll
             for (int j = 0; j < 8; ++j) x[j] = ok ? phi(x[j]) : 0.f;
-            put_row(ks, row, scol, pack8(x));
+            sw::put_row(ks + 32 * it * sw::ROW, sb, pack8(x));
             unpack8(rq[it], x);
 #pragma unroll
             for (int j = 0; j < 8; ++j) x[j] = ok ? phi(x[j]) : 0.f;
-            put_row(qs, row, scol, pack8(x));
+            sw::put_row(qs + 32 * it * sw::ROW, sb, pack8(x));
         }
         __syncthreads();
         if (c > cbeg) { CLA_LOAD(c - 1); }
 
         if (!STATE_ONLY) {
         if (!(wi == 0 && wj == 1)) {
-            f32x16 W = prod_rows(zero16(), gs, 32 * wi + l31, vs, 32 * wj + l31, 0, 4, hf);
+            f32x16 W = sw::prod_rows(zero16(), gs, bi8, vs, bj8, 0, 4);
             W = mfma(first_if(hf == 0, dd[32 * wi + l31]), first_if(hf == 0, 1.0f), W);
-            put_acc_T(wt, 32 * wj + l31, 32 * wi, W, hf, wi == wj ? l31 : 0, 64, 0.f);
-            const f32x16 A = prod_rows(zero16(), qs, 32 * wi + l31, ks, 32 * wj + l31, 0, 4, hf);
-            put_acc_T(at, 32 * wj + l31, 32 * wi, A, hf, wi == wj ? l31 : 0, 64, 0.f);
+            sw::put_acc_T(wt, bj4, 32 * wi, W, hf, wi == wj ? l31 : 0, 64, 0.f);
+            const f32x16 A = sw::prod_rows(zero16(), qs, bi8, ks, bj8, 0, 4);
+            sw::put_acc_T(at, bj4, 32 * wi, A, hf, wi == wj ? l31 : 0, 64, 0.f);
         }
         __syncthreads();
 
@@ -537,27 +565,27 @@
             f32x16 K = zero16();
 #pragma unroll 2
             for (int s = s0; s < 4; ++s)
-                K = mfma(tfrag8(qs, 16 * s, 32 * wj, lane), row8(wt, 32 * wi + l31, 16 * s + 8 * hf), K);
-            K = prod_accA(K, RT0, RT1, vs, 32 * wi + l31, hf);
+                K = mfma(sw::tfrag8(qs, tb, 16 * s, 32 * wj), sw::row8(wt, bi8, 16 * s), K);
+            K = sw::prod_accA(K, RT0, RT1, vs, bi4);
             {
                 bf16x8 hi, lo;
                 acc_frag(RTa, 0, hi, lo);
                 const bf16x8 b = first_if(hf == 0, 1.0f);
                 K = mfma_hl(hi, lo, b, K);
             }
-            put_acc_T(ok_, 32 * wi + l31, 32 * wj, K, hf, 0, 64, 0.f);
+            sw::put_acc_T(ok_, bi4, 32 * wj, K, hf, 0, 64, 0.f);
             f32x16 V = zero16();
 #pragma unroll 2
             for (int s = s0; s < 4; ++s)
-                V = mfma(tfrag8(gs, 16 * s, 32 * wj, lane), row8(at, 32 * wi + l31, 16 * s + 8 * hf), V);
-            V = prod_accA(V, R20, R21, ks, 32 * wi + l31, hf);
-            put_acc_T(ov, 32 * wi + l31, 32 * wj, V, hf, 0, 64, 0.f);
+                V = mfma(sw::tfrag8(gs, tb, 16 * s, 32 * wj), sw::row8(at, bi8, 16 * s), V);
+            V = sw::prod_accA(V, R20, R21, ks, bi4);
+            sw::put_acc_T(ov, bi4, 32 * wj, V, hf, 0, 64, 0.f);
         }
         }
 #pragma unroll 2
         for (int s = STATE_ONLY ? 2 * wi : 0; s < (STATE_ONLY ? 2 * wi + 2 : 4); ++s) {
-            const bf16x8 g0 = tfrag8(gs, 16 * s, 0, lane), g1 = tfrag8(gs, 16 * s, 32, lane);
-            const bf16x8 q0 = tfrag8(qs, 16 * s, 0, lane), q1 = tfrag8(qs, 16 * s, 32, lane);
+            const bf16x8 g0 = sw::tfrag8(gs, tb, 16 * s, 0), g1 = sw::tfrag8(gs, tb, 16 * s, 32);
+            const bf16x8 q0 = sw::tfrag8(qs, tb, 16 * s, 0), q1 = sw::tfrag8(qs, tb, 16 * s, 32);
             const bf16x8 bq = wj == 0 ? q0 : q1;
             const bf16x8 bg = wj == 0 ? g0 : g1;
             RT0 = mfma(g0, bq, RT0);
@@ -575,9 +603,9 @@
             RTa = mfma(dh, bq, RTa);
             RTa = mfma(dl, bq, RTa);
             if (STATE_ONLY) {
-                const bf16x8 bk = tfrag8(ks, 16 * s, 32 * wj, lane);
-                T0 = mfma(tfrag8(vs, 16 * s, 0, lane), bk, T0);
-                T1 = mfma(tfrag8(vs, 16 * s, 32, lane), bk, T1);
+                const bf16x8 bk = sw::tfrag8(ks, tb, 16 * s, 32 * wj);
+                T0 = mfma(sw::tfrag8(vs, tb, 16 * s, 0), bk, T0);
+                T1 = mfma(sw::tfrag8(vs, tb, 16 * s, 32), bk, T1);
                 Ta = mfma(ones0, bk, Ta);
             }
         }
@@ -598,6 +626,7 @@
     CLA_STORE(cbeg);
 #undef CLA_LOAD
 #undef CLA_STORE
+#undef CLA_FRESH
     if (csum_k) {
         float* scratch = reinterpret_cast<float*>(wt);
         colsum_store(bsk, scratch, csum_k + (((long)n * P + seg) * H + h) * D, tid, lane, w);
@@ -612,10 +641,10 @@
 
 __device__ __forceinline__ float min1(float f) { return __builtin_amdgcn_fmed3f(f, 0.0f, 1.0f); }
 
-__device__ __forceinline__ void put_acc_T_dphi(bf16_t* x, const bf16_t* f_t, int xrow, int c0, const f32x16& acc, int hf) {
+__device__ __forceinline__ void put_acc_T_dphi(bf16_t* x, const bf16_t* f_t, int x4, int c0, const f32x16& acc) {
 #pragma unroll
     for (int g = 0; g < 4; ++g) {
-        const uint2 fr = *reinterpret_cast<const uint2*>(f_t + xrow * LD + c0 + 8 * g + 4 * hf);
+        const uint2 fr = *sw::at<uint2>(f_t, x4, c0 + 8 * g);
         const float f0 = __uint_as_float(fr.x << 16), f1 = __uint_as_float(fr.x & 0xffff0000u);
         const float f2 = __uint_as_float(fr.y << 16), f3 = __uint_as_float(fr.y & 0xffff0000u);
         bf16x4 p;
@@ -623,37 +652,44 @@
         p[1] = (__bf16)(acc[4 * g + 1] * min1(f1));
         p[2] = (__bf16)(acc[4 * g + 2] * min1(f2));
         p[3] = (__bf16)(acc[4 * g + 3] * min1(f3));
-        *reinterpret_cast<uint2*>(x + xrow * LD + c0 + 8 * g + 4 * hf) = __builtin_bit_cast(uint2, p);
-    }
-}
-__device__ __forceinline__ void put_acc_T_all(bf16_t* x, int xrow, int c0, const f32x16& acc, int hf) {
+        *sw::at<uint2>(x, x4, c0 + 8 * g) = __builtin_bit_cast(uint2, p);
+    }
+}
+__device__ __forceinline__ void put_acc_T_all(bf16_t* x, int x4, int c0, const f32x16& acc) {
 #pragma unroll
     for (int g = 0; g < 4; ++g) {
         bf16x4 p;
 #pragma unroll
         for (int u = 0; u < 4; ++u) p[u] = (__bf16)acc[4 * g + u];
-        *reinterpret_cast<uint2*>(x + xrow * LD + c0 + 8 * g + 4 * hf) = __builtin_bit_cast(uint2, p);
-    }
-}
-__device__ __forceinline__ void put_acc_T_ge(bf16_t* x, int xrow, int c0, const f32x16& acc, int hf, int lo) {
+        *sw::at<uint2>(x, x4, c0 + 8 * g) = __builtin_bit_cast(uint2, p);
+    }
+}
+__device__ __forceinline__ void put_acc_T_ge(bf16_t* x, int x4, int c0, const f32x16& acc, int hf, int lo) {
 #pragma unroll
     for (int g = 0; g < 4; ++g) {
         bf16x4 p;
 #pragma unroll
         for (int u = 0; u < 4; ++u) p[u] = (__bf16)(8 * g + 4 * hf + u >= lo ? acc[4 * g + u] : 0.f);
-        *reinterpret_cast<uint2*>(x + xrow * LD + c0 + 8 * g + 4 * hf) = __builtin_bit_cast(uint2, p);
-    }
-}
-__device__ __forceinline__ f32x16 prod_rows4(const bf16_t* a_t, int arow, const bf16_t* b_t, int brow, int hf) {
-    f32x16 acc = mfma(row8(a_t, arow, 8 * hf), row8(b_t, brow, 8 * hf), zero16());
-#pragma unroll
-    for (int s = 1; s < 4; ++s) acc = mfma(row8(a_t, arow, 16 * s + 8 * hf), row8(b_t, brow, 16 * s + 8 * hf), acc);
+        *sw::at<uint2>(x, x4, c0 + 8 * g) = __builtin_bit_cast(uint2, p);
+    }
+}
+__device__ __forceinline__ f32x16 prod_rows4(const bf16_t* a_t, int a8, const bf16_t* b_t, int b8) {
+    f32x16 acc = mfma(sw::row8(a_t, a8, 0), sw::row8(b_t, b8, 0), zero16());
+#pragma unroll
+    for (int s = 1; s < 4; ++s) acc = mfma(sw::row8(a_t, a8, 16 * s), sw::row8(b_t, b8, 16 * s), acc);
     return acc;
 }
 __device__ __forceinline__ bf16x8 negate8(bf16x8 x) {
     uint4 u = __builtin_bit_cast(uint4, x);
     u.x ^= 0x80008000u; u.y ^= 0x80008000u; u.z ^= 0x80008000u; u.w ^= 0x80008000u;
     return __builtin_bit_cast(bf16x8, u);
+}
+
+__device__ __forceinline__ bf16x8 dden_frag(const bf16_t* t, int k0, int lane) {
+    const bf16_t* base = t + (k0 + 8 * (lane >> 5) + ((lane >> 2) & 3)) * 8 + 4 * (lane & 1);
+    const s16x4 a = __builtin_amdgcn_ds_read_tr16_b64_v4i16((lds_s16x4*)(base));
+    const s16x4 b = __builtin_amdgcn_ds_read_tr16_b64_v4i16((lds_s16x4*)(base + 4 * 8));
+    return __builtin_bit_cast(bf16x8, __builtin_shufflevector(a, b, 0, 1, 2, 3, 4, 5, 6, 7));
 }
 
 __global__ __launch_bounds__(512, 1) void cla_bwd_sweep_bf16_kernel(
@@ -662,7 +698,7 @@
     const float* __restrict__ fin, bf16_t* __restrict__ dq, bf16_t* __restrict__ dk, bf16_t* __restrict__ dv,
     float* __restrict__ csum_q, float* __restrict__ csum_k, float* __restrict__ csum_v, int H, int L, long ldq,
     long ldk, long ldv, long ldo, long lddo, long lddq, long lddk, long lddv) {
-    constexpr int TILE = C * LD;
+    constexpr int TILE = sw::TILE;
     __shared__ __attribute__((aligned(16))) bf16_t in_[2 * 4 * TILE];
     __shared__ __attribute__((aligned(16))) bf16_t er[2 * TILE];
     __shared__ __attribute__((aligned(16))) bf16_t es[TILE];
@@ -671,6 +707,7 @@
     __shared__ __attribute__((aligned(16))) bf16_t ok_[TILE];
     __shared__ __attribute__((aligned(16))) bf16_t ov[TILE];
     __shared__ __attribute__((aligned(16))) bf16_t oq[TILE];
+    __shared__ __attribute__((aligned(16))) bf16_t dds[2 * C * 8];
     __shared__ float dd[2][C];
     __shared__ float r1s[2][C];
     __shared__ float ksm[C];
@@ -694,6 +731,10 @@
 
     const int srow = tid >> 3, scol = (tid & 7) * 8;
     const int orow = (tid & 255) >> 3;
+    int sb = sw::base(srow, scol), osb = sw::base(orow, scol);
+    int bi8 = sw::base(32 * wi + l31, 8 * hf), bj8 = sw::base(32 * wj + l31, 8 * hf);
+    int bi4 = sw::base(32 * wi + l31, 4 * hf), bj4 = sw::base(32 * wj + l31, 4 * hf);
+    sw::TBase tb = sw::tbase(lane);
     const int nch = (L + C - 1) / C;
 
     const __amdgpu_buffer_rsrc_t qr = make_rsrc(qb, (uint32_t)(((long)(L - 1) * ldq + D) * 2));
@@ -716,16 +757,16 @@
         bf16_t* t = in_ + b * 4 * TILE;
         float dden;
         const uint4 gp = stage_g(R.g, R.o, R.z, dden);
-        put_row(t + 3 * TILE, srow, scol, gp);
+        sw::put_row(t + 3 * TILE, sb, gp);
         if ((tid & 7) == 0) {
             dd[b][srow] = dden;
             const __bf16 hh = (__bf16)dden;
             const __bf16 ll = (__bf16)(dden - (float)hh);
             const uint32_t hl = (uint32_t)__builtin_bit_cast(unsigned short, hh) |
                                 ((uint32_t)__builtin_bit_cast(unsigned short, ll) << 16);
-            put_row(t + 3 * TILE, srow, 64, make_uint4(hl, 0u, 0u, 0u));
-        }
-        put_row(t + 2 * TILE, srow, scol, R.v);
+            *reinterpret_cast<uint4*>(dds + (b * C + srow) * 8) = make_uint4(hl, 0u, 0u, 0u);
+        }
+        sw::put_row(t + 2 * TILE, sb, R.v);
         float x[8], y[8];
         unpack8(R.k, x);
         unpack8(R.q, y);
@@ -738,8 +779,8 @@
 #pragma unroll
             for (int j = 0; j < 8; ++j) x[j] = y[j] = 0.f;
         }
-        put_row(t + 1 * TILE, srow, scol, pack8(x));
-        put_row(t, srow, scol, pack8(y));
+        sw::put_row(t + 1 * TILE, sb, pack8(x));
+        sw::put_row(t, sb, pack8(y));
     };
 
     typedef float f32x8 __attribute__((ext_vector_type(8)));
@@ -761,11 +802,11 @@
             const int row = orow + 32 * it;
             const long grow = (long)c * C + row;
             if (grow < L) {
-                const uint4 a = *reinterpret_cast<const uint4*>(t0 + row * LD + scol);
+                const uint4 a = sw::get_row(t0 + 32 * it * sw::ROW, osb);
                 b0 += widen(a);
                 *reinterpret_cast<uint4*>(g0 + grow * l0 + scol) = a;
                 if (kvg) {
-                    const uint4 b = *reinterpret_cast<const uint4*>(ov + row * LD + scol);
+                    const uint4 b = sw::get_row(ov + 32 * it * sw::ROW, osb);
                     b1 += widen(b);
                     *reinterpret_cast<uint4*>(dvb + grow * lddv + scol) = b;
                 }
@@ -780,13 +821,23 @@
         for (int r = 0; r < 16; ++r) st[r] = f[(32 * wi + acc_row(r, hf)) * 64 + 32 * wj + l31];
         if (wi == 0) sa[0] = hf == 0 ? f[64 * 64 + 32 * wj + l31] : 0.f;
     } else {
-        put_acc_T_all(er, 32 * wj + l31, 32 * wi, st, hf);
+        put_acc_T_all(er, bj4, 32 * wi, st);
         if (wi == 0 && hf == 0) r1s[0][32 * wj + l31] = 0.f;
     }
-    const bf16x8 ones0 = ones_if(l31 == 0);
-    const bf16x8 one0 = first_if(hf == 0, 1.0f);
+    auto ones0 = [&]() __attribute__((always_inline)) {
+        int z = l31;
+        CWLT_SW_FRESH(z);
+        return ones_if(z == 0);
+    };
+    auto one0 = [&]() __attribute__((always_inline)) {
+        int z = hf;
+        CWLT_SW_FRESH(z);
+        return first_if(z == 0, 1.0f);
+    };
 
     auto iter = [&](int c, ChunkRegs& R, const int b) __attribute__((always_inline)) {
+        CWLT_SW_FRESH(sb); CWLT_SW_FRESH(osb); CWLT_SW_FRESH(bi8); CWLT_SW_FRESH(bj8); CWLT_SW_FRESH(bi4);
+        CWLT_SW_FRESH(bj4); CWLT_SW_FRESH(tb.b0); CWLT_SW_FRESH(tb.b4);
         if (c < nch - 1) store(c + 1, bs0, bs1);
         if (c >= 1) {
             stage(R, c - 1, 1 - b);
@@ -800,81 +851,112 @@
         __builtin_amdgcn_sched_barrier(0);
         if (kvg) {
             if (!(wi == 0 && wj == 1)) {
-                f32x16 W = prod_rows4(gs, 32 * wi + l31, vs, 32 * wj + l31, hf);
-                W = mfma(first_if(hf == 0, dden_i), one0, W);
-                if (wi == wj) put_acc_T_ge(wt, 32 * wj + l31, 32 * wi, W, hf, l31);
-                else put_acc_T_all(wt, 32 * wj + l31, 32 * wi, W, hf);
+                f32x16 W = prod_rows4(gs, bi8, vs, bj8);
+                W = mfma(first_if(hf == 0, dden_i), one0(), W);
+                if (wi == wj) put_acc_T_ge(wt, bj4, 32 * wi, W, hf, l31);
+                else put_acc_T_all(wt, bj4, 32 * wi, W);
             }
             __builtin_amdgcn_sched_barrier(0);
 #pragma unroll
             for (int s = 0; s < 4; ++s) {
-                const bf16x8 bq = tfrag8(qs, 16 * s, 32 * wj, lane);
-                st = mfma(tfrag8(gs, 16 * s, 32 * wi, lane), bq, st);
-                if (wi == 0) sa = mfma(tfrag8(gs, 16 * s, 64, lane), bq, sa);
+                const bf16x8 bq = sw::tfrag8(qs, tb, 16 * s, 32 * wj);
+                st = mfma(sw::tfrag8(gs, tb, 16 * s, 32 * wi), bq, st);
+                if (wi == 0) sa = mfma(dden_frag(dds + b * C * 8, 16 * s, lane), bq, sa);
             }
             if (c > 0) {
-                put_acc_T_all(er + (1 - b) * TILE, 32 * wj + l31, 32 * wi, st, hf);
+                put_acc_T_all(er + (1 - b) * TILE, bj4, 32 * wi, st);
                 if (wi == 0 && hf == 0) r1s[1 - b][32 * wj + l31] = sa[0] + sa[1];
             }
         } else {
             if (!(wi == 0 && wj == 1)) {
-                const f32x16 A = prod_rows4(qs, 32 * wi + l31, ks, 32 * wj + l31, hf);
-                if (wi == wj) put_acc_T_ge(at, 32 * wj + l31, 32 * wi, A, hf, l31);
-                else put_acc_T_all(at, 32 * wj + l31, 32 * wi, A, hf);
+                const f32x16 A = prod_rows4(qs, bi8, ks, bj8);
+                if (wi == wj) put_acc_T_ge(at, bj4, 32 * wi, A, hf, l31);
+                else put_acc_T_all(at, bj4, 32 * wi, A);
             }
             __builtin_amdgcn_sched_barrier(0);
             if (c == 0) {
                 st = zero16();
                 sa = zero16();
             } else {
+                const bf16x8 o0 = ones0();
 #pragma unroll
                 for (int s = 0; s < 4; ++s) {
-                    const bf16x8 nb = negate8(tfrag8(ks, 16 * s, 32 * wj, lane));
-                    st = mfma(tfrag8(vs, 16 * s, 32 * wi, lane), nb, st);
-                    if (wi == 0) sa = mfma(ones0, nb, sa);
+                    const bf16x8 nb = negate8(sw::tfrag8(ks, tb, 16 * s, 32 * wj));
+                    st = mfma(sw::tfrag8(vs, tb, 16 * s, 32 * wi), nb, st);
+                    if (wi == 0) sa = mfma(o0, nb, sa);
                 }
             }
-            put_acc_T_all(es, 32 * wj + l31, 32 * wi, st, hf);
+            put_acc_T_all(es, bj4, 32 * wi, st);
             if (wi == 0 && hf == 0) ksm[32 * wj + l31] = sa[0];
         }
         __syncthreads();
+        constexpr int FETCH_AHEAD = 1;
         if (kvg) {
             const bf16_t* rs = er + b * TILE;
-            f32x16 K = prod_rows4(rs, 32 * wj + l31, vs, 32 * wi + l31, hf);
-            K = mfma(first_if(hf == 0, r1s[b][32 * wj + l31]), one0, K);
-            f32x16 V = mfma(tfrag8(rs, 0, 32 * wj, lane), row8(ks, 32 * wi + l31, 8 * hf), zero16());
-#pragma unroll
-            for (int s = 1; s < 4; ++s)
-                V = mfma(tfrag8(rs, 16 * s, 32 * wj, lane), row8(ks, 32 * wi + l31, 16 * s + 8 * hf), V);
-            __builtin_amdgcn_sched_barrier(0);
-            if (wi == 0) {
-#pragma unroll
-                for (int s = 0; s < 2; ++s) {
-                    K = mfma(tfrag8(qs, 16 * s, 32 * wj, lane), row8(wt, 32 * wi + l31, 16 * s + 8 * hf), K);
-                    V = mfma(tfrag8(gs, 16 * s, 32 * wj, lane), row8(at, 32 * wi + l31, 16 * s + 8 * hf), V);
+            auto products = [&](auto s0c) __attribute__((always_inline)) {
+                constexpr int S0 = decltype(s0c)::value, NS = 9 + 2 * (4 - S0);
+                auto is_k = [](int i) { return i < 5 || (i >= 9 && (i - 9) % 2 == 0); };
+                auto fetch = [&](int i, bf16x8& fa, bf16x8& fb) __attribute__((always_inline)) {
+                    if (i < 4) {
+                        fa = sw::row8(rs, bj8, 16 * i);
+                        fb = sw::row8(vs, bi8, 16 * i);
+                    } else if (i == 4) {
+                        fa = first_if(hf == 0, r1s[b][32 * wj + l31]);
+                        fb = one0();
+                    } else if (i < 9) {
+                        fa = sw::tfrag8(rs, tb, 16 * (i - 5), 32 * wj);
+                        fb = sw::row8(ks, bi8, 16 * (i - 5));
+                    } else {
+                        const int k0 = 16 * (S0 + (i - 9) / 2);
+                        fa = sw::tfrag8((i - 9) % 2 == 0 ? qs : gs, tb, k0, 32 * wj);
+                        fb = sw::row8((i - 9) % 2 == 0 ? wt : at, bi8, k0);
+                    }
+                };
+                bf16x8 fa[NS], fb[NS];
+                f32x16 K = zero16(), V = zero16();
+#pragma unroll
+                for (int i = 0; i < FETCH_AHEAD; ++i) fetch(i, fa[i], fb[i]);
+#pragma unroll
+                for (int i = 0; i < NS; ++i) {
+                    if (i + FETCH_AHEAD < NS) fetch(i + FETCH_AHEAD, fa[i + FETCH_AHEAD], fb[i + FETCH_AHEAD]);
+                    __builtin_amdgcn_sched_barrier(0);
+                    if (is_k(i)) K = mfma(fa[i], fb[i], K);
+                    else V = mfma(fa[i], fb[i], V);
                 }
-            }
-#pragma unroll
-            for (int s = 2; s < 4; ++s) {
-                K = mfma(tfrag8(qs, 16 * s, 32 * wj, lane), row8(wt, 32 * wi + l31, 16 * s + 8 * hf), K);
-                V = mfma(tfrag8(gs, 16 * s, 32 * wj, lane), row8(at, 32 * wi + l31, 16 * s + 8 * hf), V);
-            }
-            __builtin_amdgcn_sched_barrier(0);
-            put_acc_T_dphi(ok_, ks, 32 * wi + l31, 32 * wj, K, hf);
-            put_acc_T_all(ov, 32 * wi + l31, 32 * wj, V, hf);
+                put_acc_T_dphi(ok_, ks, bi4, 32 * wj, K);
+                put_acc_T_all(ov, bi4, 32 * wj, V);
+            };
+            if (wi == 0) products(std::integral_constant<int, 0>{});
+            else products(std::integral_constant<int, 2>{});
         } else {
-            f32x16 Q = prod_rows4(es, 32 * wj + l31, gs, 32 * wi + l31, hf);
-            Q = mfma(first_if(hf == 0, ksm[32 * wj + l31]), first_if(hf == 0, dden_i), Q);
-            __builtin_amdgcn_sched_barrier(0);
-#pragma unroll
-            for (int s = 0; s < 2; ++s)
-                Q = mfma(tfrag8(ks, 16 * s, 32 * wj, lane), tfrag8(wt, 16 * s, 32 * wi, lane), Q);
-            if (wi == 1) {
-#pragma unroll
-                for (int s = 2; s < 4; ++s)
-                    Q = mfma(tfrag8(ks, 16 * s, 32 * wj, lane), tfrag8(wt, 16 * s, 32 * wi, lane), Q);
-            }
-            put_acc_T_dphi(oq, qs, 32 * wi + l31, 32 * wj, Q, hf);
+            auto products = [&](auto s1c) __attribute__((always_inline)) {
+                constexpr int S1 = decltype(s1c)::value, NS = 5 + S1;
+                auto fetch = [&](int i, bf16x8& fa, bf16x8& fb) __attribute__((always_inline)) {
+                    if (i < 4) {
+                        fa = sw::row8(es, bj8, 16 * i);
+                        fb = sw::row8(gs, bi8, 16 * i);
+                    } else if (i == 4) {
+                        fa = first_if(hf == 0, ksm[32 * wj + l31]);
+                        fb = first_if(hf == 0, dden_i);
+                    } else {
+                        fa = sw::tfrag8(ks, tb, 16 * (i - 5), 32 * wj);
+                        fb = sw::tfrag8(wt, tb, 16 * (i - 5), 32 * wi);
+                    }
+                };
+                bf16x8 fa[NS], fb[NS];
+                f32x16 Q = zero16();
+#pragma unroll
+                for (int i = 0; i < FETCH_AHEAD; ++i) fetch(i, fa[i], fb[i]);
+#pragma unroll
+                for (int i = 0; i < NS; ++i) {
+                    if (i + FETCH_AHEAD < NS) fetch(i + FETCH_AHEAD, fa[i + FETCH_AHEAD], fb[i + FETCH_AHEAD]);
+                    __builtin_amdgcn_sched_barrier(0);
+                    Q = mfma(fa[i], fb[i], Q);
+                }
+                put_acc_T_dphi(oq, qs, bi4, 32 * wj, Q);
+            };
+            if (wi == 0) products(std::integral_constant<int, 2>{});
+            else products(std::integral_constant<int, 4>{});
         }
         __syncthreads();
     };
diff --git a/reinforcement-learning-in-music-generation_amd/csrc/cwlt_mfma_bf16.h b/reinforcement-learning-in-music-generation_amd/csrc/cwlt_mfma_bf16.h
--- a/reinforcement-learning-in-music-generation_amd/csrc/cwlt_mfma_bf16.h
+++ b/reinforcement-learning-in-music-generation_amd/csrc/cwlt_mfma_bf16.h
@@ -131,5 +131,85 @@
             make_float4(acc[4 * g], acc[4 * g + 1], acc[4 * g + 2], acc[4 * g + 3]);
 }
 
-}
-}
+constexpr int SWZ_A0 = 0;
+constexpr int SWZ_A1 = 4;
+constexpr int SWZ_A2 = 1;
+constexpr int SWZ_A3 = 2;
+namespace sw {
+constexpr int ROW = 64;
+constexpr int TILE = C * ROW;
+__device__ __forceinline__ int swz(int row) {
+    static_assert(SWZ_A0 == 0 && SWZ_A1 == 4 && SWZ_A2 == 1 && SWZ_A3 == 2, "swz() spells these constants out");
+    return ((row & 2) << 4) | ((row & 12) << 1);
+}
+__device__ __forceinline__ int base(int row, int col) { return 2 * (row * ROW + (col ^ swz(row))); }
+template <class T>
+__device__ __forceinline__ const T* at(const bf16_t* t, int b, int cc) {
+    return reinterpret_cast<const T*>(reinterpret_cast<const char*>(t) + (b ^ (2 * cc)));
+}
+template <class T>
+__device__ __forceinline__ T* at(bf16_t* t, int b, int cc) {
+    return reinterpret_cast<T*>(reinterpret_cast<char*>(t) + (b ^ (2 * cc)));
+}
+#define CWLT_SW_FRESH(b) asm volatile("" : "+v"(b))
+
+__device__ __forceinline__ bf16x8 row8(const bf16_t* t, int b8, int k) {
+    return __builtin_bit_cast(bf16x8, *at<uint4>(t, b8, k));
+}
+__device__ __forceinline__ bf16x8 perm8(const bf16_t* t, int b4, int k0) {
+    const uint2 a = *at<uint2>(t, b4, k0);
+    const uint2 b = *at<uint2>(t, b4, k0 + 8);
+    return __builtin_bit_cast(bf16x8, make_uint4(a.x, a.y, b.x, b.y));
+}
+struct TBase {
+    int b0, b4;
+};
+__device__ __forceinline__ TBase tbase(int lane) {
+    const int row = 8 * (lane >> 5) + ((lane >> 2) & 3), col = 16 * ((lane >> 4) & 1) + 4 * (lane & 3);
+    return TBase{base(row, col), base(row + 4, col)};
+}
+__device__ __forceinline__ bf16x8 tfrag8(const bf16_t* t, const TBase& tb, int k0, int c0) {
+    const s16x4 a = __builtin_amdgcn_ds_read_tr16_b64_v4i16((lds_s16x4*)(at<s16x4>(t + k0 * ROW, tb.b0, c0)));
+    const s16x4 b = __builtin_amdgcn_ds_read_tr16_b64_v4i16((lds_s16x4*)(at<s16x4>(t + k0 * ROW, tb.b4, c0)));
+    return __builtin_bit_cast(bf16x8, __builtin_shufflevector(a, b, 0, 1, 2, 3, 4, 5, 6, 7));
+}
+__device__ __forceinline__ void put_row(bf16_t* t, int sb, uint4 v) { *at<uint4>(t, sb, 0) = v; }
+__device__ __forceinline__ uint4 get_row(const bf16_t* t, int sb) { return *at<uint4>(t, sb, 0); }
+
+__device__ __forceinline__ f32x16 prod_rows(f32x16 acc, const bf16_t* a_t, int a8, const bf16_t* b_t, int b8, int s0,
+                                            int s1) {
+#pragma unroll 2
+    for (int s = s0; s < s1; ++s) acc = mfma(row8(a_t, a8, 16 * s), row8(b_t, b8, 16 * s), acc);
+    return acc;
+}
+__device__ __forceinline__ f32x16 prod_accA(f32x16 acc, const f32x16& X0, const f32x16& X1, const bf16_t* b_t,
+                                            int b4) {
+#pragma unroll
+    for (int t = 0; t < 2; ++t) {
+        const f32x16& X = t == 0 ? X0 : X1;
+#pragma unroll
+        for (int s = 0; s < 2; ++s) {
+            bf16x8 hi, lo;
+            acc_frag(X, s, hi, lo);
+            acc = mfma_hl(hi, lo, perm8(b_t, b4, 32 * t + 16 * s), acc);
+        }
+    }
+    return acc;
+}
+__device__ __forceinline__ void put_acc_T(bf16_t* x, int x4, int c0, const f32x16& acc, int hf, int lo, int hi,
+                                          float add) {
+#pragma unroll
+    for (int g = 0; g < 4; ++g) {
+        bf16x4 p;
+#pragma unroll
+        for (int u = 0; u < 4; ++u) {
+            const int rr = 8 * g + 4 * hf + u;
+            p[u] = (__bf16)((rr >= lo && rr <= hi) ? acc[4 * g + u] + add : 0.f);
+        }
+        *at<uint2>(x, x4, c0 + 8 * g) = __builtin_bit_cast(uint2, p);
+    }
+}
+}
+
+}
+}
```

Measured after the change: 3.266 million CW-tokens/s, median of 6. About the same (+0.4%).
